# mourisl/Rcorrector

Measured on AMD Instinct MI355X. Metric: corrected reads/sec (150 bp, k=23), higher is better.
Workload: dtype u8/int32/u64

## Files before the change

rcorrector_amd/csrc/rc_correct_core.h:

```cpp
#pragma once
#include "rc_common.h"

#define RC_BS_INLINE 16
#define RC_K(P) (W::KT > 0 ? W::KT : (P).k)

struct rc_run_params {
    int k;
    int max_fix_per_k;
    double error_rate;
    int bad_qual;
    uint32_t bs[RC_BS_INLINE];
    int flags;
    const uint32_t *bs_ext;
    const uint8_t *bound_small;
};
#define RC_BOUND_SMALL 4096
RC_HD uint32_t rc_bs_lookup(const rc_run_params &P, int t)
{
    if (!P.bs[0] || t < 2) return 0;
    if (t < RC_BS_INLINE) return P.bs[t];
    if (!P.bs_ext || t >= RC_BOUND_STEPS) return 0;
    const uint32_t v = P.bs_ext[t];
    return v == RC_BOUND_NEVER ? 0 : v;
}
#define RC_PF_NO_ALT 1

struct rc_island {
    short from, to;
};
struct rc_segment {
    short from, to, lanchor, ranchor;
    int top2[2];
};

struct rc_cnt4 {
    int c0, c1, c2, c3;
};

struct rc_frame {
    uint64_t code;
    int inv;
    int pos;
    int t;
    int threshold;
    int fix_cnt;
    int bottleneck;
    rc_cnt4 cnt;
    int mask;
};

struct rc_read_state {
    unsigned char *base;
    int *counts;
    int *v;
    signed char *path;
    signed char *best;
    unsigned char *strongb;
    unsigned char *polya;
    signed char *qual;
    rc_island *isl;
    rc_segment *seg;
    uint64_t *m_a, *m_t;
    uint64_t *m_n, *m_inv;
    uint64_t *m_x;
    uint32_t *pk;
    int *spec_cnt;
    int *spec_meta;
    int *memo;
    uint64_t *spec_code;
    int *spec_inv;
    int *spec_ret;
    int *spec_keep;
    int *spec_thr;
    int *spec_mask;
    int len, kcnt;
};

#ifndef RC_SPEC
#define RC_SPEC 16
#endif
#define RC_SPEC_ENTRIES 128
#define RC_MEMO_MAX 32

struct rc_spec_state {
    int n;
    int pos;
    int dir;
};

RC_HD int rc_popc64(uint64_t x)
{
#if defined(__HIP_DEVICE_COMPILE__)
    return __popcll(x);
#else
    return __builtin_popcountll(x);
#endif
}
RC_HD int rc_ctz64(uint64_t x)
{
#if defined(__HIP_DEVICE_COMPILE__)
    return __ffsll((long long)x) - 1;
#else
    return __builtin_ctzll(x);
#endif
}
RC_HD int rc_clz64(uint64_t x)
{
#if defined(__HIP_DEVICE_COMPILE__)
    return __clzll((long long)x);
#else
    return __builtin_clzll(x);
#endif
}

RC_HD uint64_t rc_window(const uint64_t *m, int i, int n)
{
    const int w = i >> 6, sh = i & 63;
    uint64_t x = m[w] >> sh;
    if (sh) x |= m[w + 1] << (64 - sh);
    return n >= 64 ? x : (x & ((1ull << n) - 1ull));
}

RC_HD int rc_clz32(uint32_t x)
{
#if defined(__HIP_DEVICE_COMPILE__)
    return __clz((int)x);
#else
    return __builtin_clz(x);
#endif
}

template <class W>
RC_HD void rc_pack_read(W &w, rc_read_state &S)
{
    const int nwords = (S.len + 15) >> 4;
    const uint32_t *b32 = reinterpret_cast<const uint32_t *>(S.base);
    for (int wi = w.lane; wi < nwords; wi += W::STRIDE) {
        uint32_t word = 0;
        for (int q = 0; q < 4; ++q) {
            uint32_t x = b32[4 * wi + q];
            const uint32_t t = (x >> 2) & 0x01010101u;
            x = (x | t | (t << 1)) & 0x03030303u;
            word = (word << 8) | ((x * 0x40100401u) >> 24);
        }
        S.pk[wi] = word;
    }
    w.sync();
}

RC_HD uint64_t rc_code_at(const uint32_t *pk, int p, int n)
{
    const int w0 = p >> 4, sh = 2 * (p & 15);
    uint64_t x = ((uint64_t)pk[w0] << 32) | pk[w0 + 1];
    if (sh) x = (x << sh) | ((uint64_t)pk[w0 + 2] >> (32 - sh));
    return x >> (64 - 2 * n);
}

template <class W>
RC_HD void rc_build_masks(W &w, rc_read_state &S)
{
    const int nw = (S.len + 63) >> 6;
    for (int c = 0; c <= nw; ++c) {
        const int b0 = c << 6;
        const uint64_t ma = w.ballot64(b0, S.len, [&](int i) { return S.base[i] == 0; });
        const uint64_t mt = w.ballot64(b0, S.len, [&](int i) { return S.base[i] == 3; });
        const uint64_t mn = w.ballot64(b0, S.len, [&](int i) { return S.base[i] == 4; });
        const uint64_t mi = w.ballot64(b0, S.len, [&](int i) { return S.base[i] >= 4; });
        S.m_a[c] = ma;
        S.m_t[c] = mt;
        S.m_n[c] = mn;
        S.m_inv[c] = mi;
    }
    w.sync();
}

RC_HD int rc_min(int a, int b) { return a < b ? a : b; }

#define RC_U(x) (w.uni((int)(x)))
#define RC_U64(x) (w.uni64((uint64_t)(x)))

template <class W>
RC_HD int rc_screened(W &w, const rc_read_state &S, int k)
{
    (void)w;
    int n = 0, a = 0, t = 0;
    const int nw = (S.len + 63) >> 6;
    for (int c = 0; c < nw; ++c) {
        n += rc_popc64(S.m_n[c]);
        a += rc_popc64(S.m_a[c]);
        t += rc_popc64(S.m_t[c]);
    }
    return n > 5 || a > S.len - k || t > S.len - k;
}

template <class W>
RC_HD void rc_polya_flags(W &w, rc_read_state &S, int k)
{
    int thr7 = 7;
    if (k / 2 > thr7) thr7 = k / 2;
    for (int i = w.lane; i < S.kcnt; i += W::STRIDE) {
        const int a = rc_popc64(rc_window(S.m_a, i, k));
        const int t = rc_popc64(rc_window(S.m_t, i, k));
        int f = 0;
        if (a >= k - 2 || t >= k - 2) f |= 1;
        if (a >= k - thr7 || t >= k - thr7) f |= 2;
        S.polya[i] = (unsigned char)f;
    }
    w.sync();
}

template <class W>
RC_HD void rc_masked_sorted(W &w, rc_read_state &S)
{
    for (int i = w.lane; i < S.kcnt; i += W::STRIDE) S.v[i] = (S.polya[i] & 2) ? -1 : S.counts[i];
    w.sync();
    w.sort(S.v, S.kcnt);
}

template <class W>
RC_HD int rc_initial_strong(W &w, const rc_read_state &S, int *found, int *prev)
{
    const int kcnt = S.kcnt;
    for (int b0 = ((kcnt - 1) >> 6) << 6; b0 >= 0; b0 -= 64) {
        const uint64_t m = w.ballot64(b0, kcnt, [&](int i) { return i >= 1 && S.v[i] > 2 * S.v[i - 1] && S.v[i] > 10; });
        if (m) {
            const int i = b0 + 63 - rc_clz64(m);
            *found = 1;
            *prev = RC_U(S.v[i - 1]);
            return RC_U(S.v[i]);
        }
    }
    *found = 0;
    *prev = 0;
    int i = kcnt;
    for (int b0 = 0; b0 < kcnt; b0 += 64) {
        const uint64_t m = w.ballot64(b0, kcnt, [&](int j) { return S.v[j] > 0; });
        if (m) {
            i = b0 + rc_ctz64(m);
            break;
        }
    }
    return RC_U(S.v[(i + kcnt - 1) / 2]);
}

template <class W>
RC_HD int rc_front_end(W &w, rc_read_state &S, const rc_run_params &P, int *info)
{
    *info = 4;
    if (S.len < RC_K(P)) return -1;
    if (rc_screened(w, S, RC_K(P))) return -1;
    rc_polya_flags(w, S, RC_K(P));
    rc_masked_sorted(w, S);
    int found, prev;
    int strong = rc_initial_strong(w, S, &found, &prev);
    *info = (found ? 1 : 0) | ((found && prev == 2) ? 2 : 0);
    return strong;
}

struct rc_search_ctx {
    int dir;
    int start, to;
    int max_fix_cnt;
    int best_fix_cnt;
    int best_bottleneck;
    int trial_cnt;
    int top2a, top2b;
};

RC_HD int rc_pin(int x)
{
#if defined(__HIP_DEVICE_COMPILE__)
    return __builtin_amdgcn_readfirstlane(x);
#else
    return x;
#endif
}

RC_HD int rc_sel4(const rc_cnt4 &c, int idx)
{
    const int c0 = rc_pin(c.c0), c1 = rc_pin(c.c1), c2 = rc_pin(c.c2), c3 = rc_pin(c.c3);
    int r = c0;
    r = idx == 1 ? c1 : r;
    r = idx == 2 ? c2 : r;
    r = idx == 3 ? c3 : r;
    return r;
}

RC_HD int rc_candidates(const rc_cnt4 &c, int b, int threshold)
{
    int m = 0;
    if (b != 0 && c.c0 >= threshold) m |= 1;
    if (b != 1 && c.c1 >= threshold) m |= 2;
    if (b != 2 && c.c2 >= threshold) m |= 4;
    if (b != 3 && c.c3 >= threshold) m |= 8;
    return m;
}

RC_HD int rc_pos_threshold(const rc_cnt4 &cnt, int upper, double e)
{
    int mx = 0;
    mx = cnt.c0 > mx ? cnt.c0 : mx;
    mx = cnt.c1 > mx ? cnt.c1 : mx;
    mx = cnt.c2 > mx ? cnt.c2 : mx;
    mx = cnt.c3 > mx ? cnt.c3 : mx;
    int ret = rc_bound_i(mx, e);
    if (ret < 1) ret = 1;
    if (upper > ret || upper <= 0) return ret;
    return upper;
}

RC_HD int rc_max4(const rc_cnt4 &cnt)
{
    int mx = 0;
    mx = cnt.c0 > mx ? cnt.c0 : mx;
    mx = cnt.c1 > mx ? cnt.c1 : mx;
    mx = cnt.c2 > mx ? cnt.c2 : mx;
    mx = cnt.c3 > mx ? cnt.c3 : mx;
    return mx;
}

RC_HD rc_kmer rc_extend(rc_kmer km, int k, int dir, int b)
{
    return dir > 0 ? rc_append(km, k, b) : rc_prepend(km, k, b);
}

RC_HD rc_kmer rc_extend_run(const rc_read_state &S, rc_kmer kc, int k, int dir, int p0, int j)
{
    if (j <= 0) return kc;
    rc_kmer r;
    if (dir > 0) {
        r.code = ((kc.code << (2 * j)) | rc_code_at(S.pk, p0, j)) & rc_kmer_mask(k);
        const uint64_t im = rc_window(S.m_inv, p0, j);
        int inv;
        if (im)
            inv = j - 1 - (63 - rc_clz64(im));
        else
            inv = kc.inv == -1 ? -1 : kc.inv + j;
        r.inv = inv >= k ? -1 : inv;
    } else {
        const int lo = p0 - j + 1;
        if (j >= k)
            r.code = rc_code_at(S.pk, lo, k);
        else
            r.code = (kc.code >> (2 * j)) | (rc_code_at(S.pk, lo, j) << (2 * (k - j)));
        const uint64_t im = rc_window(S.m_inv, lo, j);
        int inv;
        if (im)
            inv = k - 1 - rc_ctz64(im);
        else
            inv = kc.inv == -1 ? -1 : kc.inv - j;
        r.inv = inv < 0 ? -1 : inv;
    }
    return r;
}

template <class W>
RC_HD rc_kmer rc_anchor(W &w, const rc_read_state &S, int k, int a)
{
    rc_kmer kc;
    const int w0 = a >> 4, sh = 2 * (a & 15);
    uint64_t x = ((uint64_t)(uint32_t)RC_U(S.pk[w0]) << 32) | (uint32_t)RC_U(S.pk[w0 + 1]);
    if (sh) x = (x << sh) | ((uint64_t)(uint32_t)RC_U(S.pk[w0 + 2]) >> (32 - sh));
    kc.code = x >> (64 - 2 * k);
    const int mw = a >> 6, ms = a & 63;
    uint64_t im = RC_U64(S.m_inv[mw]) >> ms;
    if (ms) im |= RC_U64(S.m_inv[mw + 1]) << (64 - ms);
    if (k < 64) im &= (1ull << k) - 1ull;
    kc.inv = im ? k - 1 - (63 - rc_clz64(im)) : -1;
    return kc;
}

template <class W>
RC_HD int rc_probe4_cached(W &w, rc_read_state &S, rc_spec_state &Z, const rc_run_params &P, rc_kmer kc, int dir, int pos, int to,
                           rc_cnt4 &cnt)
{
    const int k = RC_K(P);
    if (Z.n > 0 && Z.dir == dir) {
        const int j = (pos - Z.pos) * dir;
        if (j >= 0 && j < Z.n && RC_U64(S.spec_code[j]) == kc.code && RC_U(S.spec_inv[j]) == kc.inv) {
            cnt.c0 = RC_U(S.spec_cnt[4 * j + 0]);
            cnt.c1 = RC_U(S.spec_cnt[4 * j + 1]);
            cnt.c2 = RC_U(S.spec_cnt[4 * j + 2]);
            cnt.c3 = RC_U(S.spec_cnt[4 * j + 3]);
            return j;
        }
    }
    w.stat(3, 1);
    int n = dir > 0 ? (to - pos) : (pos - to + 1);
    if (n > RC_SPEC) n = RC_SPEC;
    if (n < 1) n = 1;
    int am = 0, ana = 0, az = 0, bz = 0;
    const int a0 = dir > 0 ? pos - k : pos + 1;
    if (!(P.flags & RC_PF_NO_ALT) && kc.inv == -1 && a0 >= 0 && a0 + k <= S.len) {
        const rc_kmer o = rc_anchor(w, S, k, a0);
        if (o.code == kc.code && o.inv == -1) {
            const uint64_t zm = w.ballot64(0, n, [&](int j) { return (dir > 0 ? S.counts[pos + j - k + 1] : S.counts[pos - j]) == 0; });
            if (zm) {
                const int z = rc_ctz64(zm), pz = pos + dir * z;
                bz = RC_U(S.base[pz]);
                const int pa = RC_U(dir > 0 ? S.polya[pz - k + 1] : S.polya[pz]);
                const int na = dir > 0 ? to - pz - 1 : pz - to;
                int mm = dir > 0 ? S.len - 1 - pz : pz;
                if (mm > k - 1) mm = k - 1;
                int m = na > mm ? na : mm;
                if (z + 1 + m > 31) m = 31 - (z + 1);
                if (4 * (z + 1) + 3 * m > RC_SPEC_ENTRIES) m = (RC_SPEC_ENTRIES - 4 * (z + 1)) / 3;
                if (bz < 4 && !RC_U(S.strongb[pz]) && !(pa & 1) && na >= 0 && na <= m && m >= 1) {
                    const uint64_t open = w.ballot64(0, na, [&](int j) {
                        const int q = pz + dir * (1 + j);
                        return !S.strongb[q] && !((dir > 0 ? S.polya[q - k + 1] : S.polya[q]) & 1);
                    });
                    if (!open) {
                        am = m;
                        ana = na;
                        az = z;
                        n = z + 1;
                    }
                }
            }
        }
    }
    w.sync();
    const int n4 = 4 * n, E = n4 + 3 * am;
    w.stat(8, E);
    w.stat(9, am > 0 ? 1 : 0);
    auto entry = [&](int e, bool *live) -> rc_kmer {
        rc_kmer km;
        km.code = 0;
        km.inv = 0;
        *live = e < E;
        if (e < n4) {
            const int j = e >> 2, c = e & 3;
            const rc_kmer kj = rc_extend_run(S, kc, k, dir, pos, j);
            if (c == 0) {
                S.spec_code[j] = kj.code;
                S.spec_inv[j] = kj.inv;
            }
            km = rc_extend(kj, k, dir, c);
        } else if (e < E) {
            const int r = e - n4;
            const int a = (r >= am ? 1 : 0) + (r >= 2 * am ? 1 : 0), j = r - a * am;
            const int ca = a + (a >= bz ? 1 : 0);
            km = rc_extend_run(S, kc, k, dir, pos, az + 2 + j);
            if (j + 1 < k) {
                const int sh = dir > 0 ? 2 * (j + 1) : 2 * (k - 1 - (j + 1));
                km.code ^= (uint64_t)(bz ^ ca) << sh;
            }
        }
        return km;
    };
    for (int e0 = 0; e0 < E; e0 += 64) {
        w.for_lanes64(e0, E, [&](int q, int) {
            bool live;
            const rc_kmer km = entry(q, &live);
            S.spec_cnt[q] = w.get(km, dir);
        });
    }
    if (w.lane == 0) {
        S.spec_meta[0] = am;
        S.spec_meta[1] = ana;
        S.spec_meta[2] = az;
    }
    w.sync();
    Z.n = n;
    Z.pos = pos;
    Z.dir = dir;
    cnt.c0 = RC_U(S.spec_cnt[0]);
    cnt.c1 = RC_U(S.spec_cnt[1]);
    cnt.c2 = RC_U(S.spec_cnt[2]);
    cnt.c3 = RC_U(S.spec_cnt[3]);
    return 0;
}

template <class W>
RC_HD int rc_alt_run(W &w, rc_read_state &S, const rc_run_params &P, int a, int dir, rc_kmer &kc, int &pos, int t, int &bottleneck,
                     bool *full)
{
    const int am = RC_U(S.spec_meta[0]), na = RC_U(S.spec_meta[1]), az = RC_U(S.spec_meta[2]);
    *full = na == 0;
    if (na == 0 || t < 1) return 0;
    uint32_t Bt = 0;
    if (dir < 0) {
        Bt = RC_U(rc_bs_lookup(P, t));
        if (!Bt) return 0;
    }
    const int eb = 4 * (az + 1) + a * am;
    const uint64_t okm = w.ballot64(0, na, [&](int j) {
        const int x = S.spec_cnt[eb + j];
        return x >= t && (uint32_t)x >= Bt;
    });
    const uint64_t notok = ~okm;
    int R = notok ? rc_ctz64(notok) : 64;
    if (R > na) R = na;
    if (R == 0) return 0;
    w.for_lanes64(0, R, [&](int j, int) { S.path[pos + dir * j] = -1; });
    bottleneck = rc_min(bottleneck, w.min_range(S.spec_cnt, eb, eb + R));
    rc_kmer nk = rc_extend_run(S, kc, RC_K(P), dir, pos, R);
    kc.code = RC_U64(nk.code);
    kc.inv = RC_U(nk.inv);
    pos += dir * R;
    *full = R == na;
    w.stat(6, 1);
    w.stat(7, R == na ? 1 : 0);
    w.sync();
    return R;
}

template <class W>
RC_HD void rc_search_terminal(W &w, rc_read_state &S, rc_search_ctx &C, const rc_spec_state &Z, int k, int pos, int t, int fix_cnt,
                              int bottleneck, int memo_a)
{
    if (bottleneck < t) ++fix_cnt;
    if (fix_cnt < C.max_fix_cnt) {
        C.top2a = bottleneck;
        C.top2b = -1;
    } else if (fix_cnt == C.max_fix_cnt) {
        if (bottleneck > C.top2a) {
            C.top2b = C.top2a;
            C.top2a = bottleneck;
        } else if (bottleneck > C.top2b) {
            C.top2b = bottleneck;
        }
    }
    if (fix_cnt < C.max_fix_cnt || (fix_cnt == C.max_fix_cnt && bottleneck > C.best_bottleneck)) {
        if (fix_cnt < C.max_fix_cnt) C.trial_cnt = -(C.max_fix_cnt - fix_cnt + 1) * RC_MAX_TRIAL;
        int lo, hi;
        if (C.dir > 0) {
            lo = C.start;
            hi = pos;
        } else {
            lo = pos + 1;
            hi = C.start + 1;
        }
        w.sync();
        for (int i = lo + w.lane; i < hi; i += W::STRIDE) S.best[i] = S.path[i];
        if (memo_a >= 0) {
            const int am = RC_U(S.spec_meta[0]), az = RC_U(S.spec_meta[2]);
            const int pz = Z.pos + C.dir * az, bz = RC_U(S.base[pz]);
            const int ca = memo_a + (memo_a >= bz ? 1 : 0);
            const int eb = 4 * (az + 1) + memo_a * am;
            const int lo_w = C.dir > 0 ? pz - k + 1 : pz - am;
            w.for_lanes64(0, am + 1, [&](int i, int) {
                int c;
                if (C.dir > 0)
                    c = i == 0 ? S.spec_cnt[4 * az + ca] : S.spec_cnt[eb + i - 1];
                else
                    c = i == am ? S.spec_cnt[4 * az + ca] : S.spec_cnt[eb + am - 1 - i];
                S.memo[4 + i] = c;
            });
            if (w.lane == 0) {
                S.memo[0] = am + 1;
                S.memo[1] = lo_w;
                S.memo[2] = pz;
                S.memo[3] = ca;
            }
        }
        w.sync();
        C.max_fix_cnt = fix_cnt;
        C.best_bottleneck = bottleneck;
        C.best_fix_cnt = 1;
    } else if (fix_cnt == C.max_fix_cnt && bottleneck == C.best_bottleneck) {
        C.best_fix_cnt += 1;
    }
}

RC_HD int rc_clamp_threshold(int ret, int upper)
{
    if (upper > ret || upper <= 0) return ret;
    return upper;
}

template <class W>
RC_HD int rc_keep_run(W &w, rc_read_state &S, const rc_run_params &P, const rc_spec_state &Z, int j0, int dir, rc_kmer &kc,
                      int &pos, int &t, int fix_cnt, int &bottleneck, int &sp)
{
    const int k = RC_K(P);
    const int n = Z.n;
    w.for_lanes64(j0, n, [&](int jj, int) {
        const int c0 = S.spec_cnt[4 * jj], c1 = S.spec_cnt[4 * jj + 1], c2 = S.spec_cnt[4 * jj + 2], c3 = S.spec_cnt[4 * jj + 3];
        int mx = 0;
        mx = c0 > mx ? c0 : mx;
        mx = c1 > mx ? c1 : mx;
        mx = c2 > mx ? c2 : mx;
        mx = c3 > mx ? c3 : mx;
        int ret = rc_bound_i(mx, P.error_rate);
        if (ret < 1) ret = 1;
        S.spec_ret[jj] = rc_clamp_threshold(ret, t);
        const int b = S.base[Z.pos + dir * jj];
        int kc2 = -1;
        kc2 = b == 0 ? c0 : kc2;
        kc2 = b == 1 ? c1 : kc2;
        kc2 = b == 2 ? c2 : kc2;
        kc2 = b == 3 ? c3 : kc2;
        S.spec_keep[jj] = kc2;
    });
    w.sync();
    if (dir > 0) {
        w.for_lanes64(j0, n, [&](int jj, int) { S.spec_thr[jj] = S.spec_ret[jj]; });
    } else {
        w.prefix_min(S.spec_ret, S.spec_thr, j0, n);
    }
    w.sync();
    const uint64_t okm = w.ballot64(j0, n, [&](int jj) { return S.spec_keep[jj] >= S.spec_thr[jj]; });
    const uint64_t notok = ~okm;
    int R = notok ? rc_ctz64(notok) : 64;
    if (R > n - j0) R = n - j0;
    w.stat(0, 1);
    w.stat(1, R);
    w.stat(2, n - j0);
    if (R == 0) return 0;
    const uint64_t fm = w.ballot64(j0, j0 + R, [&](int jj) {
        const int p2 = Z.pos + dir * jj;
        const int b = S.base[p2];
        const int pa = dir > 0 ? S.polya[p2 - k + 1] : S.polya[p2];
        int m2 = 0;
        if (!S.strongb[p2] && !(pa & 1)) {
            const int thr = S.spec_thr[jj];
            for (int c = 0; c < 4; ++c)
                if (c != b && S.spec_cnt[4 * jj + c] >= thr) m2 |= 1 << c;
        }
        S.spec_mask[jj] = m2;
        S.path[p2] = -1;
        return m2 != 0;
    });
    w.sync();
    uint64_t f2 = fm;
    while (f2) {
        const int jj = j0 + rc_ctz64(f2);
        f2 &= f2 - 1;
        rc_frame f;
        f.code = RC_U64(S.spec_code[jj]);
        f.inv = RC_U(S.spec_inv[jj]);
        f.pos = Z.pos + dir * jj;
        f.t = (dir > 0 || jj == j0) ? t : RC_U(S.spec_thr[jj - 1]);
        f.threshold = RC_U(S.spec_thr[jj]);
        f.fix_cnt = fix_cnt;
        int bb = bottleneck;
        for (int i = j0; i < jj; ++i) bb = rc_min(bb, RC_U(S.spec_keep[i]));
        f.bottleneck = bb;
        f.cnt.c0 = RC_U(S.spec_cnt[4 * jj + 0]);
        f.cnt.c1 = RC_U(S.spec_cnt[4 * jj + 1]);
        f.cnt.c2 = RC_U(S.spec_cnt[4 * jj + 2]);
        f.cnt.c3 = RC_U(S.spec_cnt[4 * jj + 3]);
        f.mask = RC_U(S.spec_mask[jj]);
        w.stack_push(sp, f);
        ++sp;
    }
    const int idx = j0 + R;
    bottleneck = rc_min(bottleneck, w.min_range(S.spec_keep, j0, idx));
    if (dir < 0) t = RC_U(S.spec_thr[idx - 1]);
    if (idx < n) {
        kc.code = RC_U64(S.spec_code[idx]);
        kc.inv = RC_U(S.spec_inv[idx]);
    } else {
        rc_kmer last;
        last.code = RC_U64(S.spec_code[idx - 1]);
        last.inv = RC_U(S.spec_inv[idx - 1]);
        kc = rc_extend(last, k, dir, RC_U(S.base[Z.pos + dir * (idx - 1)]));
    }
    pos = Z.pos + dir * idx;
    return R;
}

template <class W>
RC_HD void rc_search(W &w, rc_read_state &S, const rc_run_params &P, rc_search_ctx &C, rc_kmer kc0,
                     int t0)
{
    const int k = RC_K(P);
    const int dir = C.dir;
    int sp = 0;
    rc_kmer kc = kc0;
    int pos = C.start, t = t0, fix_cnt = 0, bottleneck = 1000000000;
    bool have = true;
    rc_spec_state Z;
    Z.n = 0;
    Z.pos = 0;
    Z.dir = dir;
    int alt_a = -1;
    auto alt_of = [&](uint64_t code, int inv, int p, int c) -> int {
        if (Z.n <= 0 || RC_U(S.spec_meta[0]) <= 0) return -1;
        const int az = RC_U(S.spec_meta[2]);
        if (p != Z.pos + dir * az || RC_U64(S.spec_code[az]) != code || RC_U(S.spec_inv[az]) != inv) return -1;
        const int bz = RC_U(S.base[p]);
        return c < bz ? c : c - 1;
    };

    for (;;) {
        w.phase(8);
        if (!have) {
            if (sp == 0) break;
            rc_frame f;
            w.stack_top(sp - 1, f);
            int c = 0;
            while (!((f.mask >> c) & 1)) ++c;
            f.mask &= ~(1 << c);
            if (f.mask == 0)
                --sp;
            else
                w.stack_set_mask(sp - 1, f.mask);
            rc_kmer fk;
            fk.code = f.code;
            fk.inv = f.inv;
            S.path[f.pos] = (signed char)c;
            w.sync();
            ++C.trial_cnt;
            alt_a = alt_of(f.code, f.inv, f.pos, c);
            kc = rc_extend(fk, k, dir, c);
            pos = f.pos + dir;
            t = dir > 0 ? f.t : f.threshold;
            fix_cnt = f.fix_cnt + (RC_U(S.base[f.pos]) < 4 ? 1 : 0);
            bottleneck = rc_min(f.bottleneck, rc_sel4(f.cnt, c));
            have = true;
        }

        if (C.trial_cnt > RC_MAX_TRIAL) {
            if (C.max_fix_cnt > 2) {
                --C.max_fix_cnt;
                C.best_fix_cnt = 0;
                C.best_bottleneck = -1;
                C.trial_cnt = 0;
            } else {
                have = false;
                continue;
            }
        }
        if (fix_cnt > C.max_fix_cnt) {
            have = false;
            alt_a = -1;
            continue;
        }
        int memo_a = -1;
        if (alt_a >= 0) {
            bool full;
            rc_alt_run(w, S, P, alt_a, dir, kc, pos, t, bottleneck, &full);
            if (full) memo_a = alt_a;
            alt_a = -1;
        }
        if (dir > 0 ? (pos >= C.to) : (pos < C.to)) {
            w.phase(14);
            rc_search_terminal(w, S, C, Z, k, pos, t, fix_cnt, bottleneck, memo_a);
            have = false;
            continue;
        }

        rc_cnt4 cnt;
        w.phase(9);
        const int j0 = rc_probe4_cached(w, S, Z, P, kc, dir, pos, C.to, cnt);
        w.phase(10);
        if (rc_keep_run(w, S, P, Z, j0, dir, kc, pos, t, fix_cnt, bottleneck, sp) > 0) {
            have = true;
            continue;
        }
        w.phase(11);
        int threshold = RC_U(rc_pos_threshold(cnt, t, P.error_rate));
        const int b = RC_U(S.base[pos]);
        const bool bvalid = b < 4;

        int mask = 0;
        {
            const int pa = RC_U(dir > 0 ? S.polya[pos - k + 1] : S.polya[pos]);
            if (!RC_U(S.strongb[pos]) && !(pa & 1)) mask = rc_candidates(cnt, b, threshold);
        }

        bool first = false;
        rc_kmer nkc = kc;
        int npos = pos, nt = t, nfix = fix_cnt, nbott = bottleneck;
        if (bvalid) {
            int c0 = rc_sel4(cnt, b);
            if (c0 >= threshold) {
                S.path[pos] = -1;
                nkc = rc_extend(kc, k, dir, b);
                npos = pos + dir;
                nt = dir > 0 ? t : threshold;
                nbott = rc_min(bottleneck, c0);
                first = true;
            } else if (threshold == 1 && t <= 2) {
                w.phase(12);
                rc_kmer tmp = rc_extend(kc, k, dir, b);
                int m = dir > 0 ? (C.to - 1 - pos) : (pos - C.to);
                if (m > k - 1) m = k - 1;
                int steps = k, i = pos;
                (void)c0;
                if (m > 0) {
                    const rc_kmer tmp0 = tmp;
                    int mc = Z.n - 1 - j0;
                    if (mc > m) mc = m;
                    int sN = 0;
                    if (mc > 0) {
                        const uint64_t hit = w.ballot64(1, mc + 1, [&](int q) { return S.spec_keep[j0 + q] >= threshold; });
                        if (hit) sN = 1 + rc_ctz64(hit);
                    }
                    if (sN == 0 && m > mc) {
                        const uint64_t hit = w.ballot64(mc + 1, m + 1, [&](int q) {
                            return w.get(rc_extend_run(S, tmp0, k, dir, pos + dir, q), dir) >= threshold;
                        });
                        w.stat(4, 1);
                        w.stat(5, m - mc);
                        if (hit) sN = mc + 1 + rc_ctz64(hit);
                    }
                    if (sN > 0) {
                        tmp = rc_extend_run(S, tmp0, k, dir, pos + dir, sN);
                        tmp.code = RC_U64(tmp.code);
                        tmp.inv = RC_U(tmp.inv);
                        i = pos + dir * sN;
                        steps = sN;
                    }
                }
                if (steps < k && (dir > 0 ? (i < C.to) : (i >= C.to))) {
                    int lo = dir > 0 ? pos : i, hi = dir > 0 ? i : pos;
                    for (int j = lo + w.lane; j <= hi; j += W::STRIDE) S.path[j] = -1;
                    nkc = tmp;
                    npos = i + dir;
                    nt = dir > 0 ? t : threshold;
                    nfix = fix_cnt + 1;
                    first = true;
                }
            }
        }

        if (!first && mask) {
            int c = 0;
            while (!((mask >> c) & 1)) ++c;
            mask &= ~(1 << c);
            S.path[pos] = (signed char)c;
            ++C.trial_cnt;
            alt_a = alt_of(kc.code, kc.inv, pos, c);
            nkc = rc_extend(kc, k, dir, c);
            npos = pos + dir;
            nt = dir > 0 ? t : threshold;
            nfix = fix_cnt + (bvalid ? 1 : 0);
            nbott = rc_min(bottleneck, rc_sel4(cnt, c));
            first = true;
        }

        if (first) {
            if (mask) {
                rc_frame f;
                f.code = kc.code;
                f.inv = kc.inv;
                f.pos = pos;
                f.t = t;
                f.threshold = threshold;
                f.fix_cnt = fix_cnt;
                f.bottleneck = bottleneck;
                f.cnt = cnt;
                f.mask = mask;
                w.stack_push(sp, f);
                ++sp;
            }
        } else {
            w.phase(13);
            rc_kmer tmp = kc;
            int i, c1 = 0;
            int thr = threshold;
            if (dir > 0) {
                for (i = pos; i < C.to; ++i) {
                    rc_cnt4 cn;
                    if (i == pos)
                        cn = cnt;
                    else
                        rc_probe4_cached(w, S, Z, P, tmp, dir, i, C.to, cn);
                    thr = RC_U(rc_pos_threshold(cn, t, P.error_rate));
                    int bb = RC_U(S.base[i]);
                    tmp = rc_append(tmp, k, bb);
                    c1 = (bb < 4) ? rc_sel4(cn, bb) : 0;
                    S.path[i] = -1;
                    if (c1 >= thr) break;
                }
                int pen = (i < S.len) ? (i - pos - k + 1) : ((i - pos) / 2);
                if (pen <= 0) pen = 1;
                nfix = fix_cnt + pen;
                if (i >= C.to) i -= 1;
                npos = i + 1;
                nt = t;
            } else {
                for (i = pos; i >= C.to; --i) {
                    rc_cnt4 cn;
                    if (i == pos)
                        cn = cnt;
                    else
                        rc_probe4_cached(w, S, Z, P, tmp, dir, i, C.to, cn);
                    thr = RC_U(rc_pos_threshold(cn, t, P.error_rate));
                    int bb = RC_U(S.base[i]);
                    tmp = rc_prepend(tmp, k, bb);
                    c1 = (bb < 4) ? rc_sel4(cn, bb) : 0;
                    S.path[i] = -1;
                    if (c1 >= thr) break;
                }
                int pen = (i >= 0) ? (pos - i - k + 1) : (pos - 1);
                if (pen <= 0) pen = 1;
                nfix = fix_cnt + pen;
                if (i <= C.to) ++i;
                npos = i - 1;
                nt = thr;
            }
            nkc = tmp;
            nbott = bottleneck;
        }
        w.sync();
        kc = nkc;
        pos = npos;
        t = nt;
        fix_cnt = nfix;
        bottleneck = nbott;
        have = true;
    }
}

template <class W>
RC_HD int rc_correct_read(W &w, rc_read_state &S, const rc_run_params &P, int pair_t, int strong0,
                          int info0)
{
    const int k = RC_K(P);
    const int len = S.len, kcnt = S.kcnt;
    if (w.lane == 0) S.memo[0] = 0;
    if (len < k) return -1;
    if (info0 & 4) return -1;
    w.trace_passed();

    int strong = strong0, trust;
    bool flag = false;
    trust = RC_U(rc_bound_i(strong, P.error_rate));
    if (info0 & 1) {
        if (strong >= 20 && (info0 & 2) && trust < 3) {
            flag = true;
            trust = 3;
        }
    }
    if (pair_t >= 1 && strong > pair_t) {
        if (!flag || pair_t < 20) trust = RC_U(rc_bound_i(pair_t, P.error_rate));
        strong = pair_t;
    }
    if (trust < 2) trust = 2;

    int iter = 0, total_fix = 0, bad_segment_cnt = 0;
    int tstart = 0, tend = 0;
    for (;;) {
        w.phase(2);
        w.trace_iter(strong, trust);
        const int allowed_fix = len;
        total_fix = 0;
        bool unfixable = false, force_next = false;
        int isl_cnt = 0, longest = -1, j = 0, i;

        for (i = w.lane; i < len; i += W::STRIDE) {
            S.strongb[i] = 0;
            S.path[i] = -1;
        }
        w.sync();

        {
            const int nwk = (kcnt + 63) >> 6;
            for (int c = 0; c <= nwk; ++c) {
                const uint64_t tm = w.ballot64(c << 6, kcnt, [&](int q) { return S.counts[q] >= strong && !(S.polya[q] & 1); });
                S.m_x[c] = tm;
            }
            w.sync();
            int *rs = S.v;
            int *re = S.v + (kcnt + 1) / 2 + 1;
            int ns = 0, ne = 0;
            for (int c = 0; c < nwk; ++c) {
                const uint64_t T = RC_U64(S.m_x[c]);
                const uint64_t prev = c ? (RC_U64(S.m_x[c - 1]) >> 63) : 0ull;
                const uint64_t next = RC_U64(S.m_x[c + 1]) & 1ull;
                uint64_t st = T & ~((T << 1) | prev);
                uint64_t en = T & ~((T >> 1) | (next << 63));
                while (st) {
                    rs[ns++] = (c << 6) + rc_ctz64(st);
                    st &= st - 1;
                }
                while (en) {
                    re[ne++] = (c << 6) + rc_ctz64(en);
                    en &= en - 1;
                }
            }
            w.sync();
            if (!(RC_U64(S.m_x[0]) & 1ull)) {
                longest = 0;
                tstart = 0;
                tend = -1;
            }
            for (int r = 0; r < ns; ++r) {
                const int f = RC_U(rs[r]), t2 = RC_U(re[r]);
                j = t2 - f + 1;
                if (j > longest) {
                    longest = j;
                    tstart = f;
                    tend = t2;
                }
                if (j >= 2) {
                    S.isl[isl_cnt].from = (short)f;
                    S.isl[isl_cnt].to = (short)t2;
                    ++isl_cnt;
                }
            }
            w.sync();
        }

        for (i = 1; i < isl_cnt; ++i) {
            int pf = RC_U(S.isl[i - 1].from), pt = RC_U(S.isl[i - 1].to), cf = RC_U(S.isl[i].from), ct = RC_U(S.isl[i].to);
            if (cf <= pt + k) {
                int len1 = pt - pf, len2 = ct - cf, overlap = pt + k - cf;
                const uint64_t weak = w.ballot64(pt + 1, cf, [&](int q) { return S.counts[q] <= 2 && S.counts[q] < trust; });
                if (!weak) continue;
                if (overlap > 3) continue;
                if (len1 < len2)
                    S.isl[i - 1].to = (short)(pt - (overlap + 1));
                else
                    S.isl[i].from = (short)(cf + (overlap + 1));
                w.sync();
            }
        }

        {
            int nb = 0, cura = 0, curb = -2;
            for (i = 0; i < isl_cnt; ++i) {
                const int f = RC_U(S.isl[i].from), tt = RC_U(S.isl[i].to);
                if (f > tt) continue;
                const int a2 = f, b2 = tt + k - 1;
                for (j = a2 + w.lane; j <= b2; j += W::STRIDE) S.strongb[j] = 1;
                if (nb > 0 && a2 <= curb + 1) {
                    if (b2 > curb) curb = b2;
                } else {
                    if (nb > 0) {
                        S.isl[nb - 1].from = (short)cura;
                        S.isl[nb - 1].to = (short)curb;
                    }
                    cura = a2;
                    curb = b2;
                    ++nb;
                }
            }
            if (nb > 0) {
                S.isl[nb - 1].from = (short)cura;
                S.isl[nb - 1].to = (short)curb;
            }
            isl_cnt = nb;
        }
        if (isl_cnt == 0) {
            S.isl[0].from = (short)tstart;
            S.isl[0].to = (short)(tend + k - 1);
            isl_cnt = 1;
        }
        w.sync();

        int seg_cnt = 0;
        {
            int f0 = RC_U(S.isl[0].from), t0 = RC_U(S.isl[0].to);
            if (f0 > 0) {
                S.seg[seg_cnt].from = 0;
                S.seg[seg_cnt].to = (short)(f0 - 1);
                S.seg[seg_cnt].lanchor = 0;
                S.seg[seg_cnt].ranchor = (short)(t0 - f0 + 1);
                ++seg_cnt;
            }
            for (i = 0; i < isl_cnt - 1; ++i) {
                int af = RC_U(S.isl[i].from), at = RC_U(S.isl[i].to), bf = RC_U(S.isl[i + 1].from), bt = RC_U(S.isl[i + 1].to);
                S.seg[seg_cnt].from = (short)(at + 1);
                S.seg[seg_cnt].to = (short)(bf - 1);
                S.seg[seg_cnt].lanchor = (short)(at - af + 1);
                S.seg[seg_cnt].ranchor = (short)(bt - bf + 1);
                ++seg_cnt;
            }
            int lf = RC_U(S.isl[i].from), lt = RC_U(S.isl[i].to);
            if (lt < len - 1) {
                S.seg[seg_cnt].from = (short)(lt + 1);
                S.seg[seg_cnt].to = (short)len;
                S.seg[seg_cnt].lanchor = (short)(lt - lf + 1);
                S.seg[seg_cnt].ranchor = 0;
                ++seg_cnt;
            }
            for (i = 0; i < seg_cnt; ++i) S.seg[i].top2[0] = S.seg[i].top2[1] = -1;
        }
        w.sync();
        w.trace_strong(S.strongb, len);

        if (longest == -1) return -1;
        if (longest == kcnt) return 0;
#if defined(RC_EXP_STOP) && RC_EXP_STOP == 3
        return 0;
#endif

        for (i = w.lane; i < len; i += W::STRIDE) S.best[i] = -1;
        w.sync();
        bad_segment_cnt = 0;
        w.phase(3);
        if (seg_cnt > 0) {
            rc_search_ctx C;
            int best_bottleneck = RC_INF;
            C.best_fix_cnt = -1;
            C.trial_cnt = 0;
            C.max_fix_cnt = allowed_fix;
            for (int si = 0; si < seg_cnt; ++si) {
                const int sf = RC_U(S.seg[si].from), st = RC_U(S.seg[si].to);
                C.top2a = C.top2b = -1;
                C.trial_cnt = 0;
                C.max_fix_cnt = (st - sf + 1) * P.max_fix_per_k / k * 2 + 1;
                if (C.max_fix_cnt < P.max_fix_per_k) C.max_fix_cnt = P.max_fix_per_k;
                C.best_bottleneck = -1;
                int a;
                if (RC_U(S.seg[si].lanchor) >= RC_U(S.seg[si].ranchor)) {
                    int extend = (st == len) ? 0 : (k - 1);
                    a = sf - k;
                    if (a < 0) return -1;
                    C.dir = 1;
                    C.start = a + k;
                    C.to = st + extend;
                } else {
                    int extend = (sf == 0) ? 0 : (k - 1);
                    a = st + 1;
                    if (a + k > len) return -1;
                    C.dir = -1;
                    C.start = a - 1;
                    C.to = sf - extend;
                }
                rc_search(w, S, P, C, rc_anchor(w, S, k, a), trust);
                w.phase(3);
                S.seg[si].top2[0] = C.top2a;
                S.seg[si].top2[1] = C.top2b;
                w.sync();
                if (C.best_bottleneck == -1) {
                    ++bad_segment_cnt;
                    continue;
                }
                if (C.best_bottleneck < best_bottleneck) best_bottleneck = C.best_bottleneck;
                if (best_bottleneck == -1) break;
                if (C.trial_cnt > RC_MAX_TRIAL) return -1;
                total_fix += C.max_fix_cnt;
            }
            int best_fix_cnt = C.best_fix_cnt;
            if (best_bottleneck != -1) {
                best_fix_cnt = 1;
                for (i = 0; i < seg_cnt; ++i)
                    if (RC_U(S.seg[i].top2[1]) >= best_bottleneck) best_fix_cnt *= 2;
            }
            if (best_bottleneck != -1 && iter == 0 &&
                RC_U(rc_less_than_bound(best_bottleneck, strong, P.error_rate) ? 1 : 0))
                force_next = true;
            if (best_fix_cnt >= 2)
                return -1;
            else if (best_fix_cnt <= 0)
                unfixable = true;
        }
        if (total_fix == 0 && force_next) return 0;
        if (total_fix > allowed_fix) unfixable = true;
        if (!unfixable && !force_next) break;
        if (trust < 10 && !force_next) return -1;

        w.phase(4);
        rc_masked_sorted(w, S);
        bool has_drop = false;
        i = 0;
        for (int b0 = ((kcnt - 1) >> 6) << 6; b0 >= 0; b0 -= 64) {
            const int st = strong;
            const uint64_t dm = w.ballot64(b0, kcnt, [&](int q) {
                if (q < 1) return false;
                const int vi = S.v[q], vp = S.v[q - 1];
                return vi <= st && ((vi > 2 * vp && vi > 10) || (vp == 0 && vi >= 5));
            });
            const uint64_t bm = dm & w.ballot64(b0, kcnt, [&](int q) { return S.v[q] < st; });
            if (bm) {
                has_drop = true;
                i = b0 + 63 - rc_clz64(bm);
                break;
            }
            if (dm) has_drop = true;
        }
        if (has_drop) {
            ++iter;
            int vi = RC_U(S.v[i]);
            trust = RC_U(rc_bound_i(vi, P.error_rate));
            strong = vi;
        } else
            break;
    }

    w.phase(5);
#if defined(RC_EXP_STOP) && RC_EXP_STOP == 4
    return total_fix;
#endif
    int cnt = 0;
    for (int b0 = 0; b0 < len; b0 += 64) {
        const uint64_t fm = w.ballot64(b0, len, [&](int q) { return S.base[q] != 4 && S.best[q] != -1; });
        if (fm) {
            w.for_lanes64(b0, len, [&](int q, int ln) {
                if ((fm >> ln) & 1ull) S.v[cnt + rc_popc64(fm & ((1ull << ln) - 1ull))] = q;
            });
            cnt += rc_popc64(fm);
        }
    }
    w.sync();
    const int badq = P.bad_qual;
    const int q0 = RC_U(S.qual[0]);
    for (int i = 1; i < cnt; ++i) {
        const int pi = RC_U(S.v[i]), pp = RC_U(S.v[i - 1]);
        if (q0 != 0 && (RC_U(S.qual[pi]) <= badq && RC_U(S.qual[pp]) <= badq)) continue;
        if (pi - pp + 1 > k) continue;
        int lo = pp - k + 1;
        if (lo < 0) lo = 0;
        if (i >= 2) {
            const int pprev = RC_U(S.v[i - 2]);
            if (lo < pprev + 1) lo = pprev + 1;
        }
        int hi = kcnt;
        if (i < cnt - 1) {
            const int pnext = RC_U(S.v[i + 1]);
            if (hi > pnext - k + 1) hi = pnext - k + 1;
        }
        uint32_t ms = 0xFFFFFFFFu, md = 0xFFFFFFFFu;
        w.for_lanes64(pp - k + 1, hi, [&](int j, int) {
            if (j < lo || j > pi) return;
            const uint32_t c = (uint32_t)S.counts[j];
            if (j + k - 1 >= pi && j <= pp)
                md = c < md ? c : md;
            else
                ms = c < ms ? c : ms;
        });
        ms = w.wave_min_u32(ms);
        md = w.wave_min_u32(md);
        if (ms == 0xFFFFFFFFu || md == 0xFFFFFFFFu) continue;
        const int min_single = (int)ms, min_double = (int)md;
        if (min_single > 1 && min_double > 1 && min_single > min_double / 2 && min_single < 2 * min_double) {
            S.best[pi] = -1;
            S.best[pp] = -1;
            for (int jj = i - 2; jj >= 0 && RC_U(S.v[jj + 1]) - RC_U(S.v[jj]) + 1 <= k; --jj) S.best[RC_U(S.v[jj])] = -1;
            while (i + 1 < cnt && RC_U(S.v[i + 1]) - RC_U(S.v[i]) + 1 <= k) {
                S.best[RC_U(S.v[i + 1])] = -1;
                ++i;
            }
            w.sync();
        }
    }

    if (total_fix > 3 && len > 10) {
        int tmp = rc_popc64(w.ballot64(0, 10, [&](int q) { return S.best[q] != -1 && S.base[q] != 4 && (int)S.qual[q] > badq; }));
        if (tmp >= 2)
            w.for_lanes64(0, 10, [&](int q, int) {
                if (S.base[q] != 4) S.best[q] = -1;
            });
        w.sync();
        tmp = rc_popc64(w.ballot64(len - 10, len, [&](int q) { return S.best[q] != -1 && S.base[q] != 4 && (int)S.qual[q] > badq; }));
        if (tmp >= 3)
            w.for_lanes64(len - 10, len, [&](int q, int) {
                if (S.base[q] != 4) S.best[q] = -1;
            });
        w.sync();
    }

    if (total_fix >= P.max_fix_per_k) {
        const int nw = (len + 63) >> 6;
        for (int c = 0; c <= nw; ++c) {
            const uint64_t f = w.ballot64(c << 6, len, [&](int q) { return S.base[q] != 4 && S.best[q] != -1; });
            const uint64_t g = f & w.ballot64(c << 6, len, [&](int q) { return (int)S.qual[q] > badq; });
            S.m_a[c] = f;
            S.m_t[c] = g;
        }
        w.sync();
        int bad = 0;
        for (int i = w.lane; i < kcnt; i += W::STRIDE)
            if (rc_popc64(rc_window(S.m_a, i, k)) + rc_popc64(rc_window(S.m_t, i, k)) > 2 * P.max_fix_per_k) bad = 1;
        if (w.reduce_add(bad)) return -1;
    }

    int ret = 0;
    for (int i = w.lane; i < len; i += W::STRIDE)
        if (S.best[i] != -1) ++ret;
    ret = w.reduce_add(ret);
    if (ret == 0 && bad_segment_cnt > 0) return -1;
    return ret;
}

template <class W>
RC_HD int rc_select_kth(W &w, const int *v, int n, int kth, uint32_t hi)
{
    uint32_t prefix = 0;
    for (int b = 31 - rc_clz32(hi | 1u); b >= 0; --b) {
        const uint32_t cand = prefix | (1u << b);
        int below = 0;
        for (int b0 = 0; b0 < n; b0 += 64) below += rc_popc64(w.ballot64(b0, n, [&](int q) { return (uint32_t)v[q] < cand; }));
        if (below <= kth) prefix = cand;
    }
    return (int)prefix;
}

template <class W>
RC_HD void rc_kmer_info(W &w, rc_read_state &S, const rc_run_params &P, int ret, int *l, int *m,
                        int *h)
{
    const int k = RC_K(P);
    *l = *m = *h = 0;
    if (S.kcnt <= 0) return;
    const int nw = (S.len + 63) >> 6;
    for (int c = 0; c <= nw; ++c) {
        uint64_t fm = 0;
        if (ret > 0) fm = w.ballot64(c << 6, S.len, [&](int q) { return S.best[q] != -1; });
        S.m_x[c] = fm;
    }
    w.sync();
    int memo_n = 0, memo_lo = 0, memo_p = 0;
    if (ret > 0) {
        memo_n = RC_U(S.memo[0]);
        if (memo_n > 0) {
            memo_lo = RC_U(S.memo[1]);
            memo_p = RC_U(S.memo[2]);
            if (RC_U(S.best[memo_p]) != RC_U(S.memo[3])) memo_n = 0;
        }
    }
    int nvalid = 0;
    uint32_t lo = 0xFFFFFFFFu, hi = 0;
    for (int b0 = 0; b0 < S.kcnt; b0 += 64) {
        const uint64_t vm = w.ballot64(b0, S.kcnt, [&](int q) {
            return (rc_window(S.m_inv, q, k) & ~rc_window(S.m_x, q, k)) == 0;
        });
        nvalid += rc_popc64(vm);
        w.for_lanes64(b0, S.kcnt, [&](int q, int ln) {
            uint32_t c = 0xFFFFFFFFu;
            if ((vm >> ln) & 1ull) {
                int cc;
                const uint64_t fw = ret > 0 ? rc_window(S.m_x, q, k) : 0ull;
                if (fw != 0) {
                    const int d = memo_p - q;
                    if (q >= memo_lo && q < memo_lo + memo_n && d >= 0 && d < k && fw == (1ull << d))
                        cc = S.memo[4 + q - memo_lo];
                    else
                        cc = w.lookup(rc_code_at(S.pk, q, k));
                } else
                    cc = S.counts[q];
                if (cc == 0) cc = 1;
                c = (uint32_t)cc;
                lo = c < lo ? c : lo;
                hi = c > hi ? c : hi;
            }
            S.v[q] = (int)c;
        });
    }
    w.sync();
    if (nvalid == 0) return;
    lo = w.wave_min_u32(lo);
    hi = w.wave_max_u32(hi);
    *l = (int)lo;
    *h = (int)hi;
    *m = rc_select_kth(w, S.v, S.kcnt, nvalid / 2, hi);
}
```

rcorrector_amd/csrc/rc_correct_kernel.h:

```cpp
#pragma once
#include <cstddef>
#include <cstdio>
#include <cstdlib>

#include "rc_internal.h"
#include "rc_device.h"

template <bool PROF, bool TRACE = false, bool SORT_REGS = true, int KT_ = 0>
struct DevWaveT {
    static const int STRIDE = 64;
    static constexpr int KT = KT_;
    int lane;
    unsigned long long t_last = 0;
    int cur_phase = 0;
    unsigned long long *acc = nullptr;
#ifdef RC_EXP_ROUNDS
    int rounds = 0;
    __device__ __forceinline__ void stat(int i, int v)
    {
        if (i == 3) rounds += v;
    }
#else
    int rounds = 0, rounds_max = 0;
    long long rounds_sum = 0;
    long long stv[10] = {0, 0, 0, 0, 0, 0, 0, 0, 0, 0};
    __device__ __forceinline__ void stat(int i, int v)
    {
        if (PROF && i == 3) rounds += v;
        if (PROF && i != 3 && i < 10) stv[i] += v;
    }
#endif
    int32_t *tr = nullptr;
    int tr_cap = 0;
    __device__ __forceinline__ void trace_passed()
    {
        if (TRACE && lane == 0) tr[0] |= 1;
    }
    __device__ __forceinline__ void trace_iter(int strong, int trust)
    {
        if (TRACE) {
            const int it = uni(tr[1]);
            if (lane == 0) {
                if (it < tr_cap) {
                    int32_t *e = tr + 2 + (size_t)it * RC_TRACE_WORDS;
                    e[0] = strong;
                    e[1] = trust;
                    e[2] = 0;
                    e[3] = 0;
                }
                tr[1] = it + 1;
            }
            sync();
        }
    }
    __device__ __forceinline__ void trace_strong(const unsigned char *strongb, int len)
    {
        if (TRACE) {
            const int it = uni(tr[1]) - 1;
            if (it >= 0 && it < tr_cap) {
                int32_t *e = tr + 2 + (size_t)it * RC_TRACE_WORDS;
                for (int c = 0; c < RC_MAX_READ_LENGTH / 64; ++c) {
                    const uint64_t m = ballot64(c << 6, len, [&](int q) { return strongb[q] != 0; });
                    if (lane == 0) {
                        e[4 + 2 * c] = (int32_t)(uint32_t)m;
                        e[5 + 2 * c] = (int32_t)(uint32_t)(m >> 32);
                    }
                }
                if (lane == 0) e[2] = 1;
            }
            sync();
        }
    }
    __device__ __forceinline__ int uni(int x) { return __builtin_amdgcn_readfirstlane(x); }
    __device__ __forceinline__ uint64_t uni64(uint64_t x)
    {
        const uint32_t lo = (uint32_t)__builtin_amdgcn_readfirstlane((int)(uint32_t)x);
        const uint32_t hi = (uint32_t)__builtin_amdgcn_readfirstlane((int)(uint32_t)(x >> 32));
        return ((uint64_t)hi << 32) | lo;
    }
    __device__ __forceinline__ void phase(int id)
    {
        if (id < 8) asm volatile("" : "+v"(lane));
        if (PROF) {
            unsigned long long t = __builtin_readcyclecounter();
            if (lane == 0) acc[cur_phase] += t - t_last;
            t_last = t;
            cur_phase = id;
        }
    }
    rc_table_view T;
    int k;
    rc_frame *stack;

    __device__ __forceinline__ void sync()
    {
        __builtin_amdgcn_fence(__ATOMIC_RELEASE, "wavefront");
        __builtin_amdgcn_wave_barrier();
        __builtin_amdgcn_fence(__ATOMIC_ACQUIRE, "wavefront");
    }

    template <class F>
    __device__ __forceinline__ uint64_t ballot64(int base, int n, F pred)
    {
        const int i = base + lane;
        bool p = false;
        if (i < n) p = pred(i);
        return __ballot(p);
    }
    template <class F>
    __device__ __forceinline__ void for_lanes64(int base, int n, F body)
    {
        const int i = base + lane;
        if (i < n) body(i, lane);
    }

    __device__ __forceinline__ int reduce_add(int x)
    {
#pragma unroll
        for (int o = 32; o > 0; o >>= 1) x += __shfl_xor(x, o, 64);
        return __builtin_amdgcn_readfirstlane(x);
    }

    template <bool MAX>
    __device__ __forceinline__ uint32_t wave_minmax_u32(uint32_t x)
    {
        auto op = [](uint32_t a, uint32_t b) { return MAX ? (a > b ? a : b) : (a < b ? a : b); };
        x = op(x, (uint32_t)__builtin_amdgcn_update_dpp(0, (int)x, 0xB1, 0xF, 0xF, true));
        x = op(x, (uint32_t)__builtin_amdgcn_update_dpp(0, (int)x, 0x4E, 0xF, 0xF, true));
        x = op(x, (uint32_t)__builtin_amdgcn_update_dpp(0, (int)x, 0x141, 0xF, 0xF, true));
        x = op(x, (uint32_t)__builtin_amdgcn_update_dpp(0, (int)x, 0x140, 0xF, 0xF, true));
        const uint32_t r0 = (uint32_t)__builtin_amdgcn_readlane((int)x, 0), r1 = (uint32_t)__builtin_amdgcn_readlane((int)x, 16);
        const uint32_t r2 = (uint32_t)__builtin_amdgcn_readlane((int)x, 32), r3 = (uint32_t)__builtin_amdgcn_readlane((int)x, 48);
        return op(op(r0, r1), op(r2, r3));
    }
    __device__ __forceinline__ uint32_t wave_min_u32(uint32_t x) { return wave_minmax_u32<false>(x); }
    __device__ __forceinline__ uint32_t wave_max_u32(uint32_t x) { return wave_minmax_u32<true>(x); }

    __device__ __forceinline__ void prefix_min(const int *in, int *out, int j0, int n)
    {
        const bool live = lane >= j0 && lane < n;
        int x = live ? in[lane] : 2147483647;
        auto step = [&](int y) { x = y < x ? y : x; };
        step(__builtin_amdgcn_update_dpp(2147483647, x, 0x111, 0xF, 0xF, false));
        step(__builtin_amdgcn_update_dpp(2147483647, x, 0x112, 0xF, 0xF, false));
        step(__builtin_amdgcn_update_dpp(2147483647, x, 0x114, 0xF, 0xF, false));
        step(__builtin_amdgcn_update_dpp(2147483647, x, 0x118, 0xF, 0xF, false));
        if (n > 16) {
            const int r0 = __builtin_amdgcn_readlane(x, 15), r1 = __builtin_amdgcn_readlane(x, 31), r2 = __builtin_amdgcn_readlane(x, 47);
            const int m01 = r0 < r1 ? r0 : r1, m012 = m01 < r2 ? m01 : r2;
            const int row = lane >> 4;
            const int before = row == 0 ? 2147483647 : (row == 1 ? r0 : (row == 2 ? m01 : m012));
            x = before < x ? before : x;
        }
        if (live) out[lane] = x;
    }
    __device__ __forceinline__ int min_range(const int *a, int lo, int hi)
    {
        const int i = lo + lane;
        const uint32_t x = i < hi ? ((uint32_t)a[i] ^ 0x80000000u) : 0xFFFFFFFFu;
        return (int)(wave_min_u32(x) ^ 0x80000000u);
    }

    uint32_t n_req = 0;
    uint32_t n_probe = 0, n_absent = 0;
    __device__ __forceinline__ int get(rc_kmer km, int dir = 0)
    {
        if (km.inv != -1) return 0;
        const uint64_t rv = rc_revcomp(km.code, KT ? KT : k);
        const uint64_t canon = rv < km.code ? rv : km.code;
        const int c = rc_table_lookup_o<true, true>(T, canon, dir > 0 ? km.code : (dir < 0 ? rv : canon), PROF ? &n_req : nullptr);
        if (PROF) {
            ++n_probe;
            n_absent += c == 0 ? 1u : 0u;
        }
        return c;
    }

    __device__ __forceinline__ int lookup(uint64_t code) { return rc_table_lookup(T, rc_canonical(code, KT ? KT : k), PROF ? &n_req : nullptr); }

    template <int E>
    __device__ __forceinline__ void bitonic_regs(int *a, int n)
    {
        int x[E];
#pragma unroll
        for (int e = 0; e < E; ++e) {
            const int g = e * 64 + lane;
            x[e] = g < n ? a[g] : 2147483647;
        }
#pragma unroll
        for (int size = 2; size <= E * 64; size <<= 1) {
#pragma unroll
            for (int stride = size >> 1; stride > 0; stride >>= 1) {
                if (stride >= 64) {
#pragma unroll
                    for (int e = 0; e < E; ++e) {
                        const int pe = e ^ (stride >> 6);
                        if (pe > e) {
                            const bool up = ((e * 64) & size) == 0;
                            const int lo = x[e] < x[pe] ? x[e] : x[pe];
                            const int hi = x[e] < x[pe] ? x[pe] : x[e];
                            x[e] = up ? lo : hi;
                            x[pe] = up ? hi : lo;
                        }
                    }
                } else {
#pragma unroll
                    for (int e = 0; e < E; ++e) {
                        const int g = e * 64 + lane;
                        const int y = __shfl_xor(x[e], stride, 64);
                        const bool up = (g & size) == 0;
                        const bool lower = (lane & stride) == 0;
                        const int lo = x[e] < y ? x[e] : y;
                        const int hi = x[e] < y ? y : x[e];
                        x[e] = (up == lower) ? lo : hi;
                    }
                }
            }
        }
        sync();
#pragma unroll
        for (int e = 0; e < E; ++e) {
            const int g = e * 64 + lane;
            if (g < n) a[g] = x[e];
        }
        sync();
    }

    __device__ __forceinline__ void sort(int *a, int n)
    {
        if (SORT_REGS) {
            if (n <= 64) return bitonic_regs<1>(a, n);
            if (n <= 128) return bitonic_regs<2>(a, n);
            if (n <= 256) return bitonic_regs<4>(a, n);
        }
        int n2 = 1;
        while (n2 < n) n2 <<= 1;
        for (int i = n + lane; i < n2; i += 64) a[i] = 2147483647;
        sync();
        for (int size = 2; size <= n2; size <<= 1) {
            for (int stride = size >> 1; stride > 0; stride >>= 1) {
                for (int t = lane; t < (n2 >> 1); t += 64) {
                    const int pos = 2 * t - (t & (stride - 1));
                    const int par = pos + stride;
                    const bool up = (pos & size) == 0;
                    const int x = a[pos], y = a[par];
                    if ((x > y) == up) {
                        a[pos] = y;
                        a[par] = x;
                    }
                }
                sync();
            }
        }
    }

    uint32_t *lstack = nullptr;
    int lstack_n = 0;
    static constexpr int FRAME_DWORDS = (int)(sizeof(rc_frame) / 4);
    __device__ __forceinline__ void stack_push(int sp, const rc_frame &f)
    {
        if (sp < lstack_n) {
            if (lane == 0) {
                uint32_t *d = lstack + sp * FRAME_DWORDS;
                d[0] = (uint32_t)f.code;
                d[1] = (uint32_t)(f.code >> 32);
                d[2] = (uint32_t)f.inv;
                d[3] = (uint32_t)f.pos;
                d[4] = (uint32_t)f.t;
                d[5] = (uint32_t)f.threshold;
                d[6] = (uint32_t)f.fix_cnt;
                d[7] = (uint32_t)f.bottleneck;
                d[8] = (uint32_t)f.cnt.c0;
                d[9] = (uint32_t)f.cnt.c1;
                d[10] = (uint32_t)f.cnt.c2;
                d[11] = (uint32_t)f.cnt.c3;
                d[12] = (uint32_t)f.mask;
            }
            sync();
            return;
        }
        if (lane == 0) stack[sp] = f;
        __threadfence_block();
    }
    __device__ __forceinline__ void stack_top(int idx, rc_frame &f)
    {
        static_assert(sizeof(rc_frame) == 56 && offsetof(rc_frame, mask) == 48, "rc_frame layout");
        uint32_t d[13];
        if (idx < lstack_n) {
            const uint32_t *p = lstack + idx * FRAME_DWORDS;
#pragma unroll
            for (int q = 0; q < 13; ++q) d[q] = p[q];
        } else {
            const uint32_t *p = reinterpret_cast<const uint32_t *>(stack + idx);
#pragma unroll
            for (int q = 0; q < 13; ++q) d[q] = __hip_atomic_load(p + q, __ATOMIC_RELAXED, __HIP_MEMORY_SCOPE_WORKGROUP);
        }
        f.code = ((uint64_t)(uint32_t)uni((int)d[1]) << 32) | (uint32_t)uni((int)d[0]);
        f.inv = uni((int)d[2]);
        f.pos = uni((int)d[3]);
        f.t = uni((int)d[4]);
        f.threshold = uni((int)d[5]);
        f.fix_cnt = uni((int)d[6]);
        f.bottleneck = uni((int)d[7]);
        f.cnt.c0 = uni((int)d[8]);
        f.cnt.c1 = uni((int)d[9]);
        f.cnt.c2 = uni((int)d[10]);
        f.cnt.c3 = uni((int)d[11]);
        f.mask = uni((int)d[12]);
    }
    __device__ __forceinline__ void stack_set_mask(int idx, int mask)
    {
        if (idx < lstack_n) {
            if (lane == 0) lstack[idx * FRAME_DWORDS + 12] = (uint32_t)mask;
            sync();
            return;
        }
        if (lane == 0) stack[idx].mask = mask;
        __threadfence_block();
    }
};
typedef DevWaveT<false> DevWave;

#ifndef RC_DEQUEUE
#define RC_DEQUEUE 8
#endif
#define RC_META_WORDS 6

struct rc_lds_layout {
    int cap, cap2;
    size_t o_counts, o_v, o_isl, o_seg, o_base, o_path, o_best, o_strongb, o_polya, o_qual, o_masks, o_spec, o_pk, o_meta, total;
    int mask_words;
};

static __host__ __device__ constexpr inline int rc_seg_capacity(int cap) { return cap <= 192 ? 20 : cap / 6 + 4; }

static __host__ __device__ constexpr inline rc_lds_layout rc_layout(int cap)
{
    rc_lds_layout L{};
    L.cap = cap;
    int c2 = 64;
    while (c2 < cap) c2 <<= 1;
    L.cap2 = c2;
    const int nseg = rc_seg_capacity(cap);
    const int nisl = cap / 3 + 2;
    size_t o = 0;
    L.mask_words = cap / 64 + 2;
    L.o_masks = o;
    o += (size_t)L.mask_words * 8 * 5;
    L.o_spec = o;
    o += (size_t)RC_SPEC_ENTRIES * 4 + (size_t)RC_SPEC * (8 + 4 + 4 * 4) + 16 + (size_t)(4 + RC_MEMO_MAX) * 4;
    L.o_pk = o;
    o += (size_t)(cap / 16 + 4) * 4;
    L.o_meta = o;
    o += (size_t)RC_DEQUEUE * RC_META_WORDS * 4;
    L.o_counts = o;
    o += (size_t)cap * 4;
    L.o_v = o;
    o += (size_t)c2 * 4;
    L.o_seg = o;
    o += (size_t)nseg * sizeof(rc_segment);
    if ((size_t)nisl * sizeof(rc_island) <= (size_t)RC_SPEC_ENTRIES * 4 + (size_t)RC_SPEC * 8) {
        L.o_isl = L.o_spec;
    } else {
        L.o_isl = o;
        o += (size_t)nisl * sizeof(rc_island);
    }
    o = (o + 15) & ~(size_t)15;
    L.o_base = o;
    o += cap;
    L.o_path = o;
    o += cap;
    L.o_best = o;
    o += cap;
    L.o_strongb = o;
    o += cap;
    L.o_polya = o;
    o += cap;
    L.o_qual = o;
    o += cap;
    L.total = (o + 15) & ~(size_t)15;
    return L;
}

__device__ __forceinline__ void rc_carve(uint8_t *lds, const rc_lds_layout &L, rc_read_state &S)
{
    S.counts = reinterpret_cast<int *>(lds + L.o_counts);
    S.v = reinterpret_cast<int *>(lds + L.o_v);
    S.seg = reinterpret_cast<rc_segment *>(lds + L.o_seg);
    S.isl = reinterpret_cast<rc_island *>(lds + L.o_isl);
    S.base = lds + L.o_base;
    S.path = reinterpret_cast<signed char *>(lds + L.o_path);
    S.best = reinterpret_cast<signed char *>(lds + L.o_best);
    S.strongb = lds + L.o_strongb;
    S.polya = lds + L.o_polya;
    S.qual = reinterpret_cast<signed char *>(lds + L.o_qual);
    uint64_t *mm = reinterpret_cast<uint64_t *>(lds + L.o_masks);
    S.m_a = mm;
    S.m_t = mm + L.mask_words;
    S.m_n = mm + 2 * L.mask_words;
    S.m_inv = mm + 3 * L.mask_words;
    S.m_x = mm + 4 * L.mask_words;
    S.pk = reinterpret_cast<uint32_t *>(lds + L.o_pk);
    S.spec_code = reinterpret_cast<uint64_t *>(lds + L.o_spec);
    S.spec_cnt = reinterpret_cast<int *>(lds + L.o_spec + RC_SPEC * 8);
    S.spec_inv = S.spec_cnt + RC_SPEC_ENTRIES;
    S.spec_ret = S.spec_inv + RC_SPEC;
    S.spec_keep = S.spec_ret + RC_SPEC;
    S.spec_thr = S.spec_keep + RC_SPEC;
    S.spec_mask = S.spec_thr + RC_SPEC;
    S.spec_meta = S.spec_mask + RC_SPEC;
    S.memo = S.spec_meta + 4;
}

struct rc_kernel_args {
    rc_table_view T;
    rc_run_params P;
    int mode;
    uint32_t n;
    uint8_t *seq;
    size_t nbytes;
    const uint8_t *qual;
    int qual_bits;
    uint32_t qual_split, qual_base2;
    const uint32_t *off;
    const int32_t *counts;
    int32_t *strong, *info;
    uint8_t *cls;
    uint8_t *cand;
    uint2 *runs;
    const uint32_t *worklist;
    const uint32_t *n_work;
    int32_t *ret, *l, *m, *h;
    rc_frame *stack;
    int stack_frames;
    uint32_t *work;
    int cap;
    int cap_class;
    unsigned long long *phase_cycles;
    int32_t *rounds_out;
    uint32_t work_stride;
    int fused_front_end;
    int32_t *trace;
    int trace_cap;
    int tier_lo, tier_hi;
    int pair_override;
};
__device__ __forceinline__ int rc_unit_max_len(const rc_kernel_args &A, uint32_t r, int len)
{
    if (A.mode == 0) return len;
    const uint32_t half = A.n >> 1, mr = A.mode == 1 ? (r < half ? r + half : r - half) : (r ^ 1u);
    const int ml = (int)(A.off[mr + 1] - A.off[mr]) - 1;
    return ml > len ? ml : len;
}
__device__ __forceinline__ bool rc_in_tier(const rc_kernel_args &A, int unit_max_len) { return unit_max_len > A.tier_lo && unit_max_len <= A.tier_hi; }

template <class W>
__device__ __forceinline__ void rc_load_read(W &w, const rc_kernel_args &A, rc_read_state &S, uint32_t o, int len, int lane, bool with_qual)
{
    S.len = len;
    S.kcnt = len >= RC_K(A.P) ? len - RC_K(A.P) + 1 : 0;
    for (int i = lane; i < len; i += 64) {
        S.base[i] = (unsigned char)rc_base_code(A.seq[o + i]);
        S.counts[i] = i < S.kcnt ? A.counts[o + i] : 0;
        if (with_qual) S.qual[i] = rc_qual_at(A.qual, A.qual_bits, A.qual_split, A.qual_base2, o + (uint32_t)i);
    }
    w.sync();
    rc_build_masks(w, S);
    rc_pack_read(w, S);
}

#ifndef RC_HEADS
#define RC_HEADS 8
#endif
#ifndef RC_K3_WAVES
#define RC_K3_WAVES 8
#endif

static __host__ __device__ constexpr int rc_k3_waves(int cap)
{
    const int by_lds = cap <= 192 ? 8 : (cap <= 320 ? 5 : 1);
    return by_lds < RC_K3_WAVES ? by_lds : RC_K3_WAVES;
}

template <int CAP, bool PROF, bool TRACE, int KT = 0, int TL = 0>
__global__ __launch_bounds__(64, rc_k3_waves(CAP)) void k_correct(rc_kernel_args A)
{
    constexpr rc_lds_layout L = rc_layout(CAP);
    __shared__ __attribute__((aligned(16))) uint8_t lds[L.total + (PROF ? 128 : 0)];
    rc_read_state S;
    rc_carve(lds, L, S);
    typedef DevWaveT<PROF, TRACE, false, KT> W;
    W w;
    w.lane = threadIdx.x;
    w.tr_cap = A.trace_cap;
    if (PROF) {
        w.acc = reinterpret_cast<unsigned long long *>(lds + L.total);
        if (w.lane < 16) w.acc[w.lane] = 0;
        w.sync();
        w.t_last = __builtin_readcyclecounter();
    }
    w.T = A.T;
    if (TL != 0) w.T.layout = 1;
    if (TL == 1) w.T.ext = 0;
    if (KT != 0) w.T.k = KT;
    w.k = A.P.k;
    w.stack = A.stack + (size_t)blockIdx.x * A.stack_frames;
    w.lstack = reinterpret_cast<uint32_t *>(S.v);
    w.lstack_n = (int)((size_t)L.cap2 * 4 / sizeof(rc_frame));
    if (PROF && w.lane == 0) atomicMin(A.phase_cycles + 8, (unsigned long long)wall_clock64());
    const int n_sections = A.n_work ? RC_WORK_CLASSES : 1;
    int section = 0;
    uint32_t n_work = A.n_work ? (uint32_t)__builtin_amdgcn_readfirstlane((int)A.n_work[0]) : A.n;
    const uint32_t *list = A.worklist;
    uint32_t *heads = A.work;
    uint32_t chunk_lo = 0, chunk_hi = 0, chunk_base = 0;
    uint32_t *meta = reinterpret_cast<uint32_t *>(lds + L.o_meta);
    int head = (int)(blockIdx.x % RC_HEADS), heads_done = 0;
    for (;;) {
        if (chunk_lo >= chunk_hi) {
            bool got = false;
            for (;;) {
                while (heads_done < RC_HEADS) {
                    const uint32_t lo = (uint32_t)(((uint64_t)n_work * (uint32_t)head) / RC_HEADS);
                    const uint32_t hi = (uint32_t)(((uint64_t)n_work * (uint32_t)(head + 1)) / RC_HEADS);
                    uint32_t r0 = hi - lo;
                    if (hi > lo) {
                        if (w.lane == 0) r0 = atomicAdd(heads + head * 32, (uint32_t)RC_DEQUEUE);
                        r0 = (uint32_t)__builtin_amdgcn_readfirstlane((int)r0);
                    }
                    if (r0 < hi - lo) {
                        chunk_lo = lo + r0;
                        chunk_hi = hi - chunk_lo > (uint32_t)RC_DEQUEUE ? chunk_lo + RC_DEQUEUE : hi;
                        got = true;
                        break;
                    }
                    head = head + 1 == RC_HEADS ? 0 : head + 1;
                    ++heads_done;
                }
                if (got || ++section >= n_sections) break;
                n_work = (uint32_t)__builtin_amdgcn_readfirstlane((int)A.n_work[section]);
                list = A.worklist + (size_t)section * A.work_stride;
                heads = A.work + section * (RC_HEADS * 32);
                head = (int)(blockIdx.x % RC_HEADS);
                heads_done = 0;
            }
            if (!got) {
                if (PROF && w.lane == 0) atomicMin(A.phase_cycles + 9, (unsigned long long)wall_clock64());
                break;
            }
            chunk_base = chunk_lo;
            if ((uint32_t)w.lane < chunk_hi - chunk_lo) {
                uint32_t ri = chunk_lo + (uint32_t)w.lane;
                if (list) ri = list[ri];
                uint32_t *mw = meta + w.lane * RC_META_WORDS;
                mw[0] = ri;
                mw[1] = A.off[ri];
                mw[2] = A.off[ri + 1];
                if (!A.fused_front_end) {
                    mw[3] = (uint32_t)A.strong[ri];
                    mw[4] = (uint32_t)A.info[ri];
                    if (A.mode == 1) {
                        const uint32_t half = A.n >> 1;
                        mw[5] = (uint32_t)A.strong[ri < half ? ri + half : ri - half];
                    } else if (A.mode == 2)
                        mw[5] = (uint32_t)A.strong[ri ^ 1u];
                }
            }
            w.sync();
        }
        const int ci = (int)(chunk_lo - chunk_base);
        ++chunk_lo;
        const uint32_t *me = meta + ci * RC_META_WORDS;
        const uint32_t r = (uint32_t)w.uni((int)me[0]);
        const uint32_t o = (uint32_t)w.uni((int)me[1]);
        w.phase(0);
        if (TRACE) {
            w.tr = A.trace + (size_t)r * (2 + (size_t)A.trace_cap * RC_TRACE_WORDS);
            if (w.lane == 0) w.tr[0] = w.tr[1] = 0;
            w.sync();
        }
#if defined(RC_EXP_STOP) && RC_EXP_STOP == 0
        if (w.lane == 0) A.ret[r] = (int)o;
        continue;
#endif
        rc_load_read(w, A, S, o, w.uni((int)(me[2] - o) - 1), w.lane, true);
#if defined(RC_EXP_STOP) && RC_EXP_STOP == 1
        if (w.lane == 0) A.ret[r] = (int)S.m_inv[0] + (int)S.pk[1] + S.counts[5] + S.qual[7];
        w.sync();
        continue;
#endif
        int strong0, info0;
        if (A.fused_front_end) {
            w.phase(1);
            strong0 = rc_front_end(w, S, A.P, &info0);
        } else {
            strong0 = w.uni((int)me[3]);
            info0 = w.uni((int)me[4]);
        }
        int pair_t = A.pair_override;
        if (A.mode != 0) pair_t = rc_min(strong0, w.uni((int)me[5]));
        w.phase(1);
        if (!A.fused_front_end && S.kcnt > 0 && !(info0 & 4)) rc_polya_flags(w, S, RC_K(A.P));
#if defined(RC_EXP_STOP) && RC_EXP_STOP == 2
        if (w.lane == 0) A.ret[r] = (int)S.polya[3] + pair_t;
        w.sync();
        continue;
#endif
        const int ret = rc_correct_read(w, S, A.P, pair_t, strong0, info0);
#if defined(RC_EXP_STOP) && (RC_EXP_STOP == 3 || RC_EXP_STOP == 4 || RC_EXP_STOP == 5)
        if (w.lane == 0) A.ret[r] = ret + S.best[3] + S.seg[0].from;
        w.sync();
        continue;
#endif
        w.phase(6);
        w.sync();
        if (ret > 0) {
            for (int i = w.lane; i < S.len; i += 64) {
                const int f = S.best[i];
                if (f != -1) {
                    A.seq[o + i] = (uint8_t)("ACGT"[f]);
                    S.base[i] = (unsigned char)f;
                }
            }
            w.sync();
            rc_pack_read(w, S);
        }
        int l, m, h;
        rc_kmer_info(w, S, A.P, ret, &l, &m, &h);
        if (w.lane == 0) {
            A.ret[r] = ret;
#ifdef RC_EXP_ROUNDS
            A.l[r] = w.rounds;
            w.rounds = 0;
#else
            A.l[r] = l;
#endif
            A.m[r] = m;
            A.h[r] = h;
        }
        w.sync();
        w.phase(7);
#ifndef RC_EXP_ROUNDS
        if (PROF) {
            if (A.rounds_out && w.lane == 0) A.rounds_out[r] = w.rounds;
            w.rounds_sum += w.rounds;
            w.rounds_max = w.rounds > w.rounds_max ? w.rounds : w.rounds_max;
            w.rounds = 0;
        }
#endif
    }
    if (PROF && w.lane == 0) {
        w.phase(7);
        for (int i = 0; i < 8; ++i) atomicAdd(A.phase_cycles + i, w.acc[i]);
        for (int i = 8; i < 16; ++i) atomicAdd(A.phase_cycles + 8 + i, w.acc[i]);
        atomicMax(A.phase_cycles + 10, (unsigned long long)wall_clock64());
#ifndef RC_EXP_ROUNDS
        atomicAdd(A.phase_cycles + 11, (unsigned long long)w.rounds_sum);
        atomicMax(A.phase_cycles + 12, (unsigned long long)w.rounds_max);
        for (int i = 0; i < 10; ++i)
            if (i != 3) atomicAdd(A.phase_cycles + 24 + i, (unsigned long long)w.stv[i]);
#endif
    }
    if (PROF) {
        const int req = w.reduce_add((int)w.n_req), prb = w.reduce_add((int)w.n_probe), abs_ = w.reduce_add((int)w.n_absent);
        if (w.lane == 0) {
            atomicAdd(A.phase_cycles + 13, (unsigned long long)(uint32_t)req);
            atomicAdd(A.phase_cycles + 14, (unsigned long long)(uint32_t)prb);
            atomicAdd(A.phase_cycles + 15, (unsigned long long)(uint32_t)abs_);
        }
    }
}

typedef void (*rc_k3_launcher)(dim3 grid, hipStream_t stream, const rc_kernel_args &A);
rc_k3_launcher rc_k3_special(int k, int layout, int ext);
#define RC_K3_SPECIAL(KT, TL)                                                                                     \
    void rc_k3_launch_##KT##_##TL(dim3 grid, hipStream_t stream, const rc_kernel_args &A)                          \
    {                                                                                                             \
        hipLaunchKernelGGL((k_correct<192, false, false, KT, TL>), grid, dim3(64), 0, stream, A);                  \
    }
```

Measured before the change: 367.2 million.

## Spill dequeue state to LDS descriptor and reload params via wave accessor to cut registers

Moves the per-wave work-queue state (chunk bounds, section/head cursor, current meta index) out of live registers into a small LDS descriptor block. It also routes run-parameter accesses through a wave-provided params accessor, so kernel arguments are re-read from their constant source instead of being held across the long correction routine. The aim is to lower VGPR/SGPR pressure in the large correction kernel and so raise occupancy or avoid spills. The cost is extra LDS reads and writes plus readfirstlane broadcasts on each read iteration.

```diff
diff --git a/rcorrector_amd/csrc/rc_correct_core.h b/rcorrector_amd/csrc/rc_correct_core.h
--- a/rcorrector_amd/csrc/rc_correct_core.h
+++ b/rcorrector_amd/csrc/rc_correct_core.h
@@ -82,6 +82,82 @@
 #define RC_SPEC_ENTRIES 128
 #define RC_MEMO_MAX 32
 
+enum {
+    RC_D_CHUNK_LO = 0,
+    RC_D_CHUNK_HI,
+    RC_D_CHUNK_BASE,
+    RC_D_QUEUE,
+    RC_D_META,
+    RC_D_WORDS = 8
+};
+RC_HD constexpr int rc_desc_queue(int section, int head, int heads_done) { return section | (head << 8) | (heads_done << 16); }
+RC_HD constexpr int rc_desc_section(int q) { return q & 0xFF; }
+RC_HD constexpr int rc_desc_head(int q) { return (q >> 8) & 0xFF; }
+RC_HD constexpr int rc_desc_heads_done(int q) { return (q >> 16) & 0xFF; }
+
+#ifndef RC_DEQUEUE
+#define RC_DEQUEUE 8
+#endif
+#define RC_META_WORDS 6
+
+struct rc_lds_layout {
+    int cap, cap2;
+    size_t o_counts, o_v, o_isl, o_seg, o_base, o_path, o_best, o_strongb, o_polya, o_qual, o_masks, o_spec, o_pk, o_meta, o_desc, total;
+    int mask_words;
+};
+
+RC_HD constexpr int rc_seg_capacity(int cap) { return cap <= 192 ? 20 : cap / 6 + 4; }
+
+RC_HD constexpr rc_lds_layout rc_layout(int cap)
+{
+    rc_lds_layout L{};
+    L.cap = cap;
+    int c2 = 64;
+    while (c2 < cap) c2 <<= 1;
+    L.cap2 = c2;
+    const int nseg = rc_seg_capacity(cap);
+    const int nisl = cap / 3 + 2;
+    size_t o = 0;
+    L.mask_words = cap / 64 + 2;
+    L.o_masks = o;
+    o += (size_t)L.mask_words * 8 * 5;
+    L.o_spec = o;
+    o += (size_t)RC_SPEC_ENTRIES * 4 + (size_t)RC_SPEC * (8 + 4 + 4 * 4) + 16 + (size_t)(4 + RC_MEMO_MAX) * 4;
+    L.o_pk = o;
+    o += (size_t)(cap / 16 + 4) * 4;
+    L.o_meta = o;
+    o += (size_t)RC_DEQUEUE * RC_META_WORDS * 4;
+    L.o_desc = o;
+    o += (size_t)RC_D_WORDS * 4;
+    L.o_counts = o;
+    o += (size_t)cap * 4;
+    L.o_v = o;
+    o += (size_t)c2 * 4;
+    L.o_seg = o;
+    o += (size_t)nseg * sizeof(rc_segment);
+    if ((size_t)nisl * sizeof(rc_island) <= (size_t)RC_SPEC_ENTRIES * 4 + (size_t)RC_SPEC * 8) {
+        L.o_isl = L.o_spec;
+    } else {
+        L.o_isl = o;
+        o += (size_t)nisl * sizeof(rc_island);
+    }
+    o = (o + 15) & ~(size_t)15;
+    L.o_base = o;
+    o += cap;
+    L.o_path = o;
+    o += cap;
+    L.o_best = o;
+    o += cap;
+    L.o_strongb = o;
+    o += cap;
+    L.o_polya = o;
+    o += cap;
+    L.o_qual = o;
+    o += cap;
+    L.total = (o + 15) & ~(size_t)15;
+    return L;
+}
+
 struct rc_spec_state {
     int n;
     int pos;
@@ -178,6 +254,18 @@
 
 #define RC_U(x) (w.uni((int)(x)))
 #define RC_U64(x) (w.uni64((uint64_t)(x)))
+
+template <class W>
+RC_HD auto rc_params_(W &w, const rc_run_params &P, int) -> decltype(w.params(P))
+{
+    return w.params(P);
+}
+template <class W>
+RC_HD const rc_run_params &rc_params_(W &, const rc_run_params &P, long)
+{
+    return P;
+}
+#define RC_P (rc_params_(w, P, 0))
 
 template <class W>
 RC_HD int rc_screened(W &w, const rc_read_state &S, int k)
@@ -391,7 +479,7 @@
     if (n < 1) n = 1;
     int am = 0, ana = 0, az = 0, bz = 0;
     const int a0 = dir > 0 ? pos - k : pos + 1;
-    if (!(P.flags & RC_PF_NO_ALT) && kc.inv == -1 && a0 >= 0 && a0 + k <= S.len) {
+    if (!(RC_P.flags & RC_PF_NO_ALT) && kc.inv == -1 && a0 >= 0 && a0 + k <= S.len) {
         const rc_kmer o = rc_anchor(w, S, k, a0);
         if (o.code == kc.code && o.inv == -1) {
             const uint64_t zm = w.ballot64(0, n, [&](int j) { return (dir > 0 ? S.counts[pos + j - k + 1] : S.counts[pos - j]) == 0; });
@@ -481,7 +569,7 @@
     if (na == 0 || t < 1) return 0;
     uint32_t Bt = 0;
     if (dir < 0) {
-        Bt = RC_U(rc_bs_lookup(P, t));
+        Bt = RC_U(rc_bs_lookup(RC_P, t));
         if (!Bt) return 0;
     }
     const int eb = 4 * (az + 1) + a * am;
@@ -583,7 +671,7 @@
         mx = c1 > mx ? c1 : mx;
         mx = c2 > mx ? c2 : mx;
         mx = c3 > mx ? c3 : mx;
-        int ret = rc_bound_i(mx, P.error_rate);
+        int ret = rc_bound_i(mx, RC_P.error_rate);
         if (ret < 1) ret = 1;
         S.spec_ret[jj] = rc_clamp_threshold(ret, t);
         const int b = S.base[Z.pos + dir * jj];
@@ -752,7 +840,7 @@
             continue;
         }
         w.phase(11);
-        int threshold = RC_U(rc_pos_threshold(cnt, t, P.error_rate));
+        int threshold = RC_U(rc_pos_threshold(cnt, t, RC_P.error_rate));
         const int b = RC_U(S.base[pos]);
         const bool bvalid = b < 4;
 
@@ -860,7 +948,7 @@
                         cn = cnt;
                     else
                         rc_probe4_cached(w, S, Z, P, tmp, dir, i, C.to, cn);
-                    thr = RC_U(rc_pos_threshold(cn, t, P.error_rate));
+                    thr = RC_U(rc_pos_threshold(cn, t, RC_P.error_rate));
                     int bb = RC_U(S.base[i]);
                     tmp = rc_append(tmp, k, bb);
                     c1 = (bb < 4) ? rc_sel4(cn, bb) : 0;
@@ -880,7 +968,7 @@
                         cn = cnt;
                     else
                         rc_probe4_cached(w, S, Z, P, tmp, dir, i, C.to, cn);
-                    thr = RC_U(rc_pos_threshold(cn, t, P.error_rate));
+                    thr = RC_U(rc_pos_threshold(cn, t, RC_P.error_rate));
                     int bb = RC_U(S.base[i]);
                     tmp = rc_prepend(tmp, k, bb);
                     c1 = (bb < 4) ? rc_sel4(cn, bb) : 0;
@@ -920,7 +1008,7 @@
 
     int strong = strong0, trust;
     bool flag = false;
-    trust = RC_U(rc_bound_i(strong, P.error_rate));
+    trust = RC_U(rc_bound_i(strong, RC_P.error_rate));
     if (info0 & 1) {
         if (strong >= 20 && (info0 & 2) && trust < 3) {
             flag = true;
@@ -928,7 +1016,7 @@
         }
     }
     if (pair_t >= 1 && strong > pair_t) {
-        if (!flag || pair_t < 20) trust = RC_U(rc_bound_i(pair_t, P.error_rate));
+        if (!flag || pair_t < 20) trust = RC_U(rc_bound_i(pair_t, RC_P.error_rate));
         strong = pair_t;
     }
     if (trust < 2) trust = 2;
@@ -1095,8 +1183,8 @@
                 const int sf = RC_U(S.seg[si].from), st = RC_U(S.seg[si].to);
                 C.top2a = C.top2b = -1;
                 C.trial_cnt = 0;
-                C.max_fix_cnt = (st - sf + 1) * P.max_fix_per_k / k * 2 + 1;
-                if (C.max_fix_cnt < P.max_fix_per_k) C.max_fix_cnt = P.max_fix_per_k;
+                C.max_fix_cnt = (st - sf + 1) * RC_P.max_fix_per_k / k * 2 + 1;
+                if (C.max_fix_cnt < RC_P.max_fix_per_k) C.max_fix_cnt = RC_P.max_fix_per_k;
                 C.best_bottleneck = -1;
                 int a;
                 if (RC_U(S.seg[si].lanchor) >= RC_U(S.seg[si].ranchor)) {
@@ -1135,7 +1223,7 @@
                     if (RC_U(S.seg[i].top2[1]) >= best_bottleneck) best_fix_cnt *= 2;
             }
             if (best_bottleneck != -1 && iter == 0 &&
-                RC_U(rc_less_than_bound(best_bottleneck, strong, P.error_rate) ? 1 : 0))
+                RC_U(rc_less_than_bound(best_bottleneck, strong, RC_P.error_rate) ? 1 : 0))
                 force_next = true;
             if (best_fix_cnt >= 2)
                 return -1;
@@ -1169,7 +1257,7 @@
         if (has_drop) {
             ++iter;
             int vi = RC_U(S.v[i]);
-            trust = RC_U(rc_bound_i(vi, P.error_rate));
+            trust = RC_U(rc_bound_i(vi, RC_P.error_rate));
             strong = vi;
         } else
             break;
@@ -1190,7 +1278,7 @@
         }
     }
     w.sync();
-    const int badq = P.bad_qual;
+    const int badq = RC_P.bad_qual;
     const int q0 = RC_U(S.qual[0]);
     for (int i = 1; i < cnt; ++i) {
         const int pi = RC_U(S.v[i]), pp = RC_U(S.v[i - 1]);
@@ -1247,7 +1335,7 @@
         w.sync();
     }
 
-    if (total_fix >= P.max_fix_per_k) {
+    if (total_fix >= RC_P.max_fix_per_k) {
         const int nw = (len + 63) >> 6;
         for (int c = 0; c <= nw; ++c) {
             const uint64_t f = w.ballot64(c << 6, len, [&](int q) { return S.base[q] != 4 && S.best[q] != -1; });
@@ -1258,7 +1346,7 @@
         w.sync();
         int bad = 0;
         for (int i = w.lane; i < kcnt; i += W::STRIDE)
-            if (rc_popc64(rc_window(S.m_a, i, k)) + rc_popc64(rc_window(S.m_t, i, k)) > 2 * P.max_fix_per_k) bad = 1;
+            if (rc_popc64(rc_window(S.m_a, i, k)) + rc_popc64(rc_window(S.m_t, i, k)) > 2 * RC_P.max_fix_per_k) bad = 1;
         if (w.reduce_add(bad)) return -1;
     }
 
diff --git a/rcorrector_amd/csrc/rc_correct_kernel.h b/rcorrector_amd/csrc/rc_correct_kernel.h
--- a/rcorrector_amd/csrc/rc_correct_kernel.h
+++ b/rcorrector_amd/csrc/rc_correct_kernel.h
@@ -5,412 +5,6 @@
 
 #include "rc_internal.h"
 #include "rc_device.h"
-
-template <bool PROF, bool TRACE = false, bool SORT_REGS = true, int KT_ = 0>
-struct DevWaveT {
-    static const int STRIDE = 64;
-    static constexpr int KT = KT_;
-    int lane;
-    unsigned long long t_last = 0;
-    int cur_phase = 0;
-    unsigned long long *acc = nullptr;
-#ifdef RC_EXP_ROUNDS
-    int rounds = 0;
-    __device__ __forceinline__ void stat(int i, int v)
-    {
-        if (i == 3) rounds += v;
-    }
-#else
-    int rounds = 0, rounds_max = 0;
-    long long rounds_sum = 0;
-    long long stv[10] = {0, 0, 0, 0, 0, 0, 0, 0, 0, 0};
-    __device__ __forceinline__ void stat(int i, int v)
-    {
-        if (PROF && i == 3) rounds += v;
-        if (PROF && i != 3 && i < 10) stv[i] += v;
-    }
-#endif
-    int32_t *tr = nullptr;
-    int tr_cap = 0;
-    __device__ __forceinline__ void trace_passed()
-    {
-        if (TRACE && lane == 0) tr[0] |= 1;
-    }
-    __device__ __forceinline__ void trace_iter(int strong, int trust)
-    {
-        if (TRACE) {
-            const int it = uni(tr[1]);
-            if (lane == 0) {
-                if (it < tr_cap) {
-                    int32_t *e = tr + 2 + (size_t)it * RC_TRACE_WORDS;
-                    e[0] = strong;
-                    e[1] = trust;
-                    e[2] = 0;
-                    e[3] = 0;
-                }
-                tr[1] = it + 1;
-            }
-            sync();
-        }
-    }
-    __device__ __forceinline__ void trace_strong(const unsigned char *strongb, int len)
-    {
-        if (TRACE) {
-            const int it = uni(tr[1]) - 1;
-            if (it >= 0 && it < tr_cap) {
-                int32_t *e = tr + 2 + (size_t)it * RC_TRACE_WORDS;
-                for (int c = 0; c < RC_MAX_READ_LENGTH / 64; ++c) {
-                    const uint64_t m = ballot64(c << 6, len, [&](int q) { return strongb[q] != 0; });
-                    if (lane == 0) {
-                        e[4 + 2 * c] = (int32_t)(uint32_t)m;
-                        e[5 + 2 * c] = (int32_t)(uint32_t)(m >> 32);
-                    }
-                }
-                if (lane == 0) e[2] = 1;
-            }
-            sync();
-        }
-    }
-    __device__ __forceinline__ int uni(int x) { return __builtin_amdgcn_readfirstlane(x); }
-    __device__ __forceinline__ uint64_t uni64(uint64_t x)
-    {
-        const uint32_t lo = (uint32_t)__builtin_amdgcn_readfirstlane((int)(uint32_t)x);
-        const uint32_t hi = (uint32_t)__builtin_amdgcn_readfirstlane((int)(uint32_t)(x >> 32));
-        return ((uint64_t)hi << 32) | lo;
-    }
-    __device__ __forceinline__ void phase(int id)
-    {
-        if (id < 8) asm volatile("" : "+v"(lane));
-        if (PROF) {
-            unsigned long long t = __builtin_readcyclecounter();
-            if (lane == 0) acc[cur_phase] += t - t_last;
-            t_last = t;
-            cur_phase = id;
-        }
-    }
-    rc_table_view T;
-    int k;
-    rc_frame *stack;
-
-    __device__ __forceinline__ void sync()
-    {
-        __builtin_amdgcn_fence(__ATOMIC_RELEASE, "wavefront");
-        __builtin_amdgcn_wave_barrier();
-        __builtin_amdgcn_fence(__ATOMIC_ACQUIRE, "wavefront");
-    }
-
-    template <class F>
-    __device__ __forceinline__ uint64_t ballot64(int base, int n, F pred)
-    {
-        const int i = base + lane;
-        bool p = false;
-        if (i < n) p = pred(i);
-        return __ballot(p);
-    }
-    template <class F>
-    __device__ __forceinline__ void for_lanes64(int base, int n, F body)
-    {
-        const int i = base + lane;
-        if (i < n) body(i, lane);
-    }
-
-    __device__ __forceinline__ int reduce_add(int x)
-    {
-#pragma unroll
-        for (int o = 32; o > 0; o >>= 1) x += __shfl_xor(x, o, 64);
-        return __builtin_amdgcn_readfirstlane(x);
-    }
-
-    template <bool MAX>
-    __device__ __forceinline__ uint32_t wave_minmax_u32(uint32_t x)
-    {
-        auto op = [](uint32_t a, uint32_t b) { return MAX ? (a > b ? a : b) : (a < b ? a : b); };
-        x = op(x, (uint32_t)__builtin_amdgcn_update_dpp(0, (int)x, 0xB1, 0xF, 0xF, true));
-        x = op(x, (uint32_t)__builtin_amdgcn_update_dpp(0, (int)x, 0x4E, 0xF, 0xF, true));
-        x = op(x, (uint32_t)__builtin_amdgcn_update_dpp(0, (int)x, 0x141, 0xF, 0xF, true));
-        x = op(x, (uint32_t)__builtin_amdgcn_update_dpp(0, (int)x, 0x140, 0xF, 0xF, true));
-        const uint32_t r0 = (uint32_t)__builtin_amdgcn_readlane((int)x, 0), r1 = (uint32_t)__builtin_amdgcn_readlane((int)x, 16);
-        const uint32_t r2 = (uint32_t)__builtin_amdgcn_readlane((int)x, 32), r3 = (uint32_t)__builtin_amdgcn_readlane((int)x, 48);
-        return op(op(r0, r1), op(r2, r3));
-    }
-    __device__ __forceinline__ uint32_t wave_min_u32(uint32_t x) { return wave_minmax_u32<false>(x); }
-    __device__ __forceinline__ uint32_t wave_max_u32(uint32_t x) { return wave_minmax_u32<true>(x); }
-
-    __device__ __forceinline__ void prefix_min(const int *in, int *out, int j0, int n)
-    {
-        const bool live = lane >= j0 && lane < n;
-        int x = live ? in[lane] : 2147483647;
-        auto step = [&](int y) { x = y < x ? y : x; };
-        step(__builtin_amdgcn_update_dpp(2147483647, x, 0x111, 0xF, 0xF, false));
-        step(__builtin_amdgcn_update_dpp(2147483647, x, 0x112, 0xF, 0xF, false));
-        step(__builtin_amdgcn_update_dpp(2147483647, x, 0x114, 0xF, 0xF, false));
-        step(__builtin_amdgcn_update_dpp(2147483647, x, 0x118, 0xF, 0xF, false));
-        if (n > 16) {
-            const int r0 = __builtin_amdgcn_readlane(x, 15), r1 = __builtin_amdgcn_readlane(x, 31), r2 = __builtin_amdgcn_readlane(x, 47);
-            const int m01 = r0 < r1 ? r0 : r1, m012 = m01 < r2 ? m01 : r2;
-            const int row = lane >> 4;
-            const int before = row == 0 ? 2147483647 : (row == 1 ? r0 : (row == 2 ? m01 : m012));
-            x = before < x ? before : x;
-        }
-        if (live) out[lane] = x;
-    }
-    __device__ __forceinline__ int min_range(const int *a, int lo, int hi)
-    {
-        const int i = lo + lane;
-        const uint32_t x = i < hi ? ((uint32_t)a[i] ^ 0x80000000u) : 0xFFFFFFFFu;
-        return (int)(wave_min_u32(x) ^ 0x80000000u);
-    }
-
-    uint32_t n_req = 0;
-    uint32_t n_probe = 0, n_absent = 0;
-    __device__ __forceinline__ int get(rc_kmer km, int dir = 0)
-    {
-        if (km.inv != -1) return 0;
-        const uint64_t rv = rc_revcomp(km.code, KT ? KT : k);
-        const uint64_t canon = rv < km.code ? rv : km.code;
-        const int c = rc_table_lookup_o<true, true>(T, canon, dir > 0 ? km.code : (dir < 0 ? rv : canon), PROF ? &n_req : nullptr);
-        if (PROF) {
-            ++n_probe;
-            n_absent += c == 0 ? 1u : 0u;
-        }
-        return c;
-    }
-
-    __device__ __forceinline__ int lookup(uint64_t code) { return rc_table_lookup(T, rc_canonical(code, KT ? KT : k), PROF ? &n_req : nullptr); }
-
-    template <int E>
-    __device__ __forceinline__ void bitonic_regs(int *a, int n)
-    {
-        int x[E];
-#pragma unroll
-        for (int e = 0; e < E; ++e) {
-            const int g = e * 64 + lane;
-            x[e] = g < n ? a[g] : 2147483647;
-        }
-#pragma unroll
-        for (int size = 2; size <= E * 64; size <<= 1) {
-#pragma unroll
-            for (int stride = size >> 1; stride > 0; stride >>= 1) {
-                if (stride >= 64) {
-#pragma unroll
-                    for (int e = 0; e < E; ++e) {
-                        const int pe = e ^ (stride >> 6);
-                        if (pe > e) {
-                            const bool up = ((e * 64) & size) == 0;
-                            const int lo = x[e] < x[pe] ? x[e] : x[pe];
-                            const int hi = x[e] < x[pe] ? x[pe] : x[e];
-                            x[e] = up ? lo : hi;
-                            x[pe] = up ? hi : lo;
-                        }
-                    }
-                } else {
-#pragma unroll
-                    for (int e = 0; e < E; ++e) {
-                        const int g = e * 64 + lane;
-                        const int y = __shfl_xor(x[e], stride, 64);
-                        const bool up = (g & size) == 0;
-                        const bool lower = (lane & stride) == 0;
-                        const int lo = x[e] < y ? x[e] : y;
-                        const int hi = x[e] < y ? y : x[e];
-                        x[e] = (up == lower) ? lo : hi;
-                    }
-                }
-            }
-        }
-        sync();
-#pragma unroll
-        for (int e = 0; e < E; ++e) {
-            const int g = e * 64 + lane;
-            if (g < n) a[g] = x[e];
-        }
-        sync();
-    }
-
-    __device__ __forceinline__ void sort(int *a, int n)
-    {
-        if (SORT_REGS) {
-            if (n <= 64) return bitonic_regs<1>(a, n);
-            if (n <= 128) return bitonic_regs<2>(a, n);
-            if (n <= 256) return bitonic_regs<4>(a, n);
-        }
-        int n2 = 1;
-        while (n2 < n) n2 <<= 1;
-        for (int i = n + lane; i < n2; i += 64) a[i] = 2147483647;
-        sync();
-        for (int size = 2; size <= n2; size <<= 1) {
-            for (int stride = size >> 1; stride > 0; stride >>= 1) {
-                for (int t = lane; t < (n2 >> 1); t += 64) {
-                    const int pos = 2 * t - (t & (stride - 1));
-                    const int par = pos + stride;
-                    const bool up = (pos & size) == 0;
-                    const int x = a[pos], y = a[par];
-                    if ((x > y) == up) {
-                        a[pos] = y;
-                        a[par] = x;
-                    }
-                }
-                sync();
-            }
-        }
-    }
-
-    uint32_t *lstack = nullptr;
-    int lstack_n = 0;
-    static constexpr int FRAME_DWORDS = (int)(sizeof(rc_frame) / 4);
-    __device__ __forceinline__ void stack_push(int sp, const rc_frame &f)
-    {
-        if (sp < lstack_n) {
-            if (lane == 0) {
-                uint32_t *d = lstack + sp * FRAME_DWORDS;
-                d[0] = (uint32_t)f.code;
-                d[1] = (uint32_t)(f.code >> 32);
-                d[2] = (uint32_t)f.inv;
-                d[3] = (uint32_t)f.pos;
-                d[4] = (uint32_t)f.t;
-                d[5] = (uint32_t)f.threshold;
-                d[6] = (uint32_t)f.fix_cnt;
-                d[7] = (uint32_t)f.bottleneck;
-                d[8] = (uint32_t)f.cnt.c0;
-                d[9] = (uint32_t)f.cnt.c1;
-                d[10] = (uint32_t)f.cnt.c2;
-                d[11] = (uint32_t)f.cnt.c3;
-                d[12] = (uint32_t)f.mask;
-            }
-            sync();
-            return;
-        }
-        if (lane == 0) stack[sp] = f;
-        __threadfence_block();
-    }
-    __device__ __forceinline__ void stack_top(int idx, rc_frame &f)
-    {
-        static_assert(sizeof(rc_frame) == 56 && offsetof(rc_frame, mask) == 48, "rc_frame layout");
-        uint32_t d[13];
-        if (idx < lstack_n) {
-            const uint32_t *p = lstack + idx * FRAME_DWORDS;
-#pragma unroll
-            for (int q = 0; q < 13; ++q) d[q] = p[q];
-        } else {
-            const uint32_t *p = reinterpret_cast<const uint32_t *>(stack + idx);
-#pragma unroll
-            for (int q = 0; q < 13; ++q) d[q] = __hip_atomic_load(p + q, __ATOMIC_RELAXED, __HIP_MEMORY_SCOPE_WORKGROUP);
-        }
-        f.code = ((uint64_t)(uint32_t)uni((int)d[1]) << 32) | (uint32_t)uni((int)d[0]);
-        f.inv = uni((int)d[2]);
-        f.pos = uni((int)d[3]);
-        f.t = uni((int)d[4]);
-        f.threshold = uni((int)d[5]);
-        f.fix_cnt = uni((int)d[6]);
-        f.bottleneck = uni((int)d[7]);
-        f.cnt.c0 = uni((int)d[8]);
-        f.cnt.c1 = uni((int)d[9]);
-        f.cnt.c2 = uni((int)d[10]);
-        f.cnt.c3 = uni((int)d[11]);
-        f.mask = uni((int)d[12]);
-    }
-    __device__ __forceinline__ void stack_set_mask(int idx, int mask)
-    {
-        if (idx < lstack_n) {
-            if (lane == 0) lstack[idx * FRAME_DWORDS + 12] = (uint32_t)mask;
-            sync();
-            return;
-        }
-        if (lane == 0) stack[idx].mask = mask;
-        __threadfence_block();
-    }
-};
-typedef DevWaveT<false> DevWave;
-
-#ifndef RC_DEQUEUE
-#define RC_DEQUEUE 8
-#endif
-#define RC_META_WORDS 6
-
-struct rc_lds_layout {
-    int cap, cap2;
-    size_t o_counts, o_v, o_isl, o_seg, o_base, o_path, o_best, o_strongb, o_polya, o_qual, o_masks, o_spec, o_pk, o_meta, total;
-    int mask_words;
-};
-
-static __host__ __device__ constexpr inline int rc_seg_capacity(int cap) { return cap <= 192 ? 20 : cap / 6 + 4; }
-
-static __host__ __device__ constexpr inline rc_lds_layout rc_layout(int cap)
-{
-    rc_lds_layout L{};
-    L.cap = cap;
-    int c2 = 64;
-    while (c2 < cap) c2 <<= 1;
-    L.cap2 = c2;
-    const int nseg = rc_seg_capacity(cap);
-    const int nisl = cap / 3 + 2;
-    size_t o = 0;
-    L.mask_words = cap / 64 + 2;
-    L.o_masks = o;
-    o += (size_t)L.mask_words * 8 * 5;
-    L.o_spec = o;
-    o += (size_t)RC_SPEC_ENTRIES * 4 + (size_t)RC_SPEC * (8 + 4 + 4 * 4) + 16 + (size_t)(4 + RC_MEMO_MAX) * 4;
-    L.o_pk = o;
-    o += (size_t)(cap / 16 + 4) * 4;
-    L.o_meta = o;
-    o += (size_t)RC_DEQUEUE * RC_META_WORDS * 4;
-    L.o_counts = o;
-    o += (size_t)cap * 4;
-    L.o_v = o;
-    o += (size_t)c2 * 4;
-    L.o_seg = o;
-    o += (size_t)nseg * sizeof(rc_segment);
-    if ((size_t)nisl * sizeof(rc_island) <= (size_t)RC_SPEC_ENTRIES * 4 + (size_t)RC_SPEC * 8) {
-        L.o_isl = L.o_spec;
-    } else {
-        L.o_isl = o;
-        o += (size_t)nisl * sizeof(rc_island);
-    }
-    o = (o + 15) & ~(size_t)15;
-    L.o_base = o;
-    o += cap;
-    L.o_path = o;
-    o += cap;
-    L.o_best = o;
-    o += cap;
-    L.o_strongb = o;
-    o += cap;
-    L.o_polya = o;
-    o += cap;
-    L.o_qual = o;
-    o += cap;
-    L.total = (o + 15) & ~(size_t)15;
-    return L;
-}
-
-__device__ __forceinline__ void rc_carve(uint8_t *lds, const rc_lds_layout &L, rc_read_state &S)
-{
-    S.counts = reinterpret_cast<int *>(lds + L.o_counts);
-    S.v = reinterpret_cast<int *>(lds + L.o_v);
-    S.seg = reinterpret_cast<rc_segment *>(lds + L.o_seg);
-    S.isl = reinterpret_cast<rc_island *>(lds + L.o_isl);
-    S.base = lds + L.o_base;
-    S.path = reinterpret_cast<signed char *>(lds + L.o_path);
-    S.best = reinterpret_cast<signed char *>(lds + L.o_best);
-    S.strongb = lds + L.o_strongb;
-    S.polya = lds + L.o_polya;
-    S.qual = reinterpret_cast<signed char *>(lds + L.o_qual);
-    uint64_t *mm = reinterpret_cast<uint64_t *>(lds + L.o_masks);
-    S.m_a = mm;
-    S.m_t = mm + L.mask_words;
-    S.m_n = mm + 2 * L.mask_words;
-    S.m_inv = mm + 3 * L.mask_words;
-    S.m_x = mm + 4 * L.mask_words;
-    S.pk = reinterpret_cast<uint32_t *>(lds + L.o_pk);
-    S.spec_code = reinterpret_cast<uint64_t *>(lds + L.o_spec);
-    S.spec_cnt = reinterpret_cast<int *>(lds + L.o_spec + RC_SPEC * 8);
-    S.spec_inv = S.spec_cnt + RC_SPEC_ENTRIES;
-    S.spec_ret = S.spec_inv + RC_SPEC;
-    S.spec_keep = S.spec_ret + RC_SPEC;
-    S.spec_thr = S.spec_keep + RC_SPEC;
-    S.spec_mask = S.spec_thr + RC_SPEC;
-    S.spec_meta = S.spec_mask + RC_SPEC;
-    S.memo = S.spec_meta + 4;
-}
 
 struct rc_kernel_args {
     rc_table_view T;
@@ -445,6 +39,388 @@
     int tier_lo, tier_hi;
     int pair_override;
 };
+
+template <bool PROF, bool TRACE = false, bool SORT_REGS = true, int KT_ = 0, bool KARG = false, int TL_ = 0>
+struct DevWaveT {
+    static const int STRIDE = 64;
+    static constexpr int KT = KT_;
+    int lane;
+    typedef const __attribute__((address_space(4))) rc_kernel_args *karg_ptr;
+    __device__ __forceinline__ karg_ptr args() const
+    {
+        karg_ptr p = (karg_ptr)__builtin_amdgcn_kernarg_segment_ptr();
+        asm volatile("" : "+s"(p));
+        return p;
+    }
+    __device__ __forceinline__ const rc_run_params &params(const rc_run_params &P) const
+    {
+        if (!KARG) return P;
+        return *(const rc_run_params *)&args()->P;
+    }
+    __device__ __forceinline__ rc_table_view table() const
+    {
+        if (!KARG) return T;
+        karg_ptr a = args();
+        rc_table_view t;
+        t.buckets = a->T.buckets;
+        t.nb_home = a->T.nb_home;
+        t.nbuckets_alloc = a->T.nbuckets_alloc;
+        t.layout = TL_ != 0 ? 1 : a->T.layout;
+        t.k = KT != 0 ? KT : a->T.k;
+        t.ext = TL_ == 1 ? 0 : a->T.ext;
+        t.filter = a->T.filter;
+        t.filter_words = a->T.filter_words;
+        t.filter_kind = a->T.filter_kind;
+        t.filter_all = a->T.filter_all;
+        return t;
+    }
+    __device__ __forceinline__ int run_k() const { return KT ? KT : (KARG ? args()->P.k : k); }
+    __device__ __forceinline__ rc_frame *hbm_stack() const
+    {
+        if (!KARG) return stack;
+        karg_ptr a = args();
+        return a->stack + (size_t)blockIdx.x * a->stack_frames;
+    }
+    unsigned long long t_last = 0;
+    int cur_phase = 0;
+    unsigned long long *acc = nullptr;
+#ifdef RC_EXP_ROUNDS
+    int rounds = 0;
+    __device__ __forceinline__ void stat(int i, int v)
+    {
+        if (i == 3) rounds += v;
+    }
+#else
+    int rounds = 0, rounds_max = 0;
+    long long rounds_sum = 0;
+    long long stv[10] = {0, 0, 0, 0, 0, 0, 0, 0, 0, 0};
+    __device__ __forceinline__ void stat(int i, int v)
+    {
+        if (PROF && i == 3) rounds += v;
+        if (PROF && i != 3 && i < 10) stv[i] += v;
+    }
+#endif
+    int32_t *tr = nullptr;
+    int tr_cap = 0;
+    __device__ __forceinline__ void trace_passed()
+    {
+        if (TRACE && lane == 0) tr[0] |= 1;
+    }
+    __device__ __forceinline__ void trace_iter(int strong, int trust)
+    {
+        if (TRACE) {
+            const int it = uni(tr[1]);
+            if (lane == 0) {
+                if (it < tr_cap) {
+                    int32_t *e = tr + 2 + (size_t)it * RC_TRACE_WORDS;
+                    e[0] = strong;
+                    e[1] = trust;
+                    e[2] = 0;
+                    e[3] = 0;
+                }
+                tr[1] = it + 1;
+            }
+            sync();
+        }
+    }
+    __device__ __forceinline__ void trace_strong(const unsigned char *strongb, int len)
+    {
+        if (TRACE) {
+            const int it = uni(tr[1]) - 1;
+            if (it >= 0 && it < tr_cap) {
+                int32_t *e = tr + 2 + (size_t)it * RC_TRACE_WORDS;
+                for (int c = 0; c < RC_MAX_READ_LENGTH / 64; ++c) {
+                    const uint64_t m = ballot64(c << 6, len, [&](int q) { return strongb[q] != 0; });
+                    if (lane == 0) {
+                        e[4 + 2 * c] = (int32_t)(uint32_t)m;
+                        e[5 + 2 * c] = (int32_t)(uint32_t)(m >> 32);
+                    }
+                }
+                if (lane == 0) e[2] = 1;
+            }
+            sync();
+        }
+    }
+    __device__ __forceinline__ int uni(int x) { return __builtin_amdgcn_readfirstlane(x); }
+    __device__ __forceinline__ uint64_t uni64(uint64_t x)
+    {
+        const uint32_t lo = (uint32_t)__builtin_amdgcn_readfirstlane((int)(uint32_t)x);
+        const uint32_t hi = (uint32_t)__builtin_amdgcn_readfirstlane((int)(uint32_t)(x >> 32));
+        return ((uint64_t)hi << 32) | lo;
+    }
+    __device__ __forceinline__ void phase(int id)
+    {
+        if (id < 8) asm volatile("" : "+v"(lane));
+        if (PROF) {
+            unsigned long long t = __builtin_readcyclecounter();
+            if (lane == 0) acc[cur_phase] += t - t_last;
+            t_last = t;
+            cur_phase = id;
+        }
+    }
+    rc_table_view T;
+    int k;
+    rc_frame *stack;
+
+    __device__ __forceinline__ void sync()
+    {
+        __builtin_amdgcn_fence(__ATOMIC_RELEASE, "wavefront");
+        __builtin_amdgcn_wave_barrier();
+        __builtin_amdgcn_fence(__ATOMIC_ACQUIRE, "wavefront");
+    }
+
+    template <class F>
+    __device__ __forceinline__ uint64_t ballot64(int base, int n, F pred)
+    {
+        const int i = base + lane;
+        bool p = false;
+        if (i < n) p = pred(i);
+        return __ballot(p);
+    }
+    template <class F>
+    __device__ __forceinline__ void for_lanes64(int base, int n, F body)
+    {
+        const int i = base + lane;
+        if (i < n) body(i, lane);
+    }
+
+    __device__ __forceinline__ int reduce_add(int x)
+    {
+#pragma unroll
+        for (int o = 32; o > 0; o >>= 1) x += __shfl_xor(x, o, 64);
+        return __builtin_amdgcn_readfirstlane(x);
+    }
+
+    template <bool MAX>
+    __device__ __forceinline__ uint32_t wave_minmax_u32(uint32_t x)
+    {
+        auto op = [](uint32_t a, uint32_t b) { return MAX ? (a > b ? a : b) : (a < b ? a : b); };
+        x = op(x, (uint32_t)__builtin_amdgcn_update_dpp(0, (int)x, 0xB1, 0xF, 0xF, true));
+        x = op(x, (uint32_t)__builtin_amdgcn_update_dpp(0, (int)x, 0x4E, 0xF, 0xF, true));
+        x = op(x, (uint32_t)__builtin_amdgcn_update_dpp(0, (int)x, 0x141, 0xF, 0xF, true));
+        x = op(x, (uint32_t)__builtin_amdgcn_update_dpp(0, (int)x, 0x140, 0xF, 0xF, true));
+        const uint32_t r0 = (uint32_t)__builtin_amdgcn_readlane((int)x, 0), r1 = (uint32_t)__builtin_amdgcn_readlane((int)x, 16);
+        const uint32_t r2 = (uint32_t)__builtin_amdgcn_readlane((int)x, 32), r3 = (uint32_t)__builtin_amdgcn_readlane((int)x, 48);
+        return op(op(r0, r1), op(r2, r3));
+    }
+    __device__ __forceinline__ uint32_t wave_min_u32(uint32_t x) { return wave_minmax_u32<false>(x); }
+    __device__ __forceinline__ uint32_t wave_max_u32(uint32_t x) { return wave_minmax_u32<true>(x); }
+
+    __device__ __forceinline__ void prefix_min(const int *in, int *out, int j0, int n)
+    {
+        const bool live = lane >= j0 && lane < n;
+        int x = live ? in[lane] : 2147483647;
+        auto step = [&](int y) { x = y < x ? y : x; };
+        step(__builtin_amdgcn_update_dpp(2147483647, x, 0x111, 0xF, 0xF, false));
+        step(__builtin_amdgcn_update_dpp(2147483647, x, 0x112, 0xF, 0xF, false));
+        step(__builtin_amdgcn_update_dpp(2147483647, x, 0x114, 0xF, 0xF, false));
+        step(__builtin_amdgcn_update_dpp(2147483647, x, 0x118, 0xF, 0xF, false));
+        if (n > 16) {
+            const int r0 = __builtin_amdgcn_readlane(x, 15), r1 = __builtin_amdgcn_readlane(x, 31), r2 = __builtin_amdgcn_readlane(x, 47);
+            const int m01 = r0 < r1 ? r0 : r1, m012 = m01 < r2 ? m01 : r2;
+            const int row = lane >> 4;
+            const int before = row == 0 ? 2147483647 : (row == 1 ? r0 : (row == 2 ? m01 : m012));
+            x = before < x ? before : x;
+        }
+        if (live) out[lane] = x;
+    }
+    __device__ __forceinline__ int min_range(const int *a, int lo, int hi)
+    {
+        const int i = lo + lane;
+        const uint32_t x = i < hi ? ((uint32_t)a[i] ^ 0x80000000u) : 0xFFFFFFFFu;
+        return (int)(wave_min_u32(x) ^ 0x80000000u);
+    }
+
+    uint32_t n_req = 0;
+    uint32_t n_probe = 0, n_absent = 0;
+    __device__ __forceinline__ int get(rc_kmer km, int dir = 0)
+    {
+        if (km.inv != -1) return 0;
+        const uint64_t rv = rc_revcomp(km.code, run_k());
+        const uint64_t canon = rv < km.code ? rv : km.code;
+        const int c = rc_table_lookup_o<true, true>(table(), canon, dir > 0 ? km.code : (dir < 0 ? rv : canon), PROF ? &n_req : nullptr);
+        if (PROF) {
+            ++n_probe;
+            n_absent += c == 0 ? 1u : 0u;
+        }
+        return c;
+    }
+
+    __device__ __forceinline__ int lookup(uint64_t code) { return rc_table_lookup(table(), rc_canonical(code, run_k()), PROF ? &n_req : nullptr); }
+
+    template <int E>
+    __device__ __forceinline__ void bitonic_regs(int *a, int n)
+    {
+        int x[E];
+#pragma unroll
+        for (int e = 0; e < E; ++e) {
+            const int g = e * 64 + lane;
+            x[e] = g < n ? a[g] : 2147483647;
+        }
+#pragma unroll
+        for (int size = 2; size <= E * 64; size <<= 1) {
+#pragma unroll
+            for (int stride = size >> 1; stride > 0; stride >>= 1) {
+                if (stride >= 64) {
+#pragma unroll
+                    for (int e = 0; e < E; ++e) {
+                        const int pe = e ^ (stride >> 6);
+                        if (pe > e) {
+                            const bool up = ((e * 64) & size) == 0;
+                            const int lo = x[e] < x[pe] ? x[e] : x[pe];
+                            const int hi = x[e] < x[pe] ? x[pe] : x[e];
+                            x[e] = up ? lo : hi;
+                            x[pe] = up ? hi : lo;
+                        }
+                    }
+                } else {
+#pragma unroll
+                    for (int e = 0; e < E; ++e) {
+                        const int g = e * 64 + lane;
+                        const int y = __shfl_xor(x[e], stride, 64);
+                        const bool up = (g & size) == 0;
+                        const bool lower = (lane & stride) == 0;
+                        const int lo = x[e] < y ? x[e] : y;
+                        const int hi = x[e] < y ? y : x[e];
+                        x[e] = (up == lower) ? lo : hi;
+                    }
+                }
+            }
+        }
+        sync();
+#pragma unroll
+        for (int e = 0; e < E; ++e) {
+            const int g = e * 64 + lane;
+            if (g < n) a[g] = x[e];
+        }
+        sync();
+    }
+
+    __device__ __forceinline__ void sort(int *a, int n)
+    {
+        if (SORT_REGS) {
+            if (n <= 64) return bitonic_regs<1>(a, n);
+            if (n <= 128) return bitonic_regs<2>(a, n);
+            if (n <= 256) return bitonic_regs<4>(a, n);
+        }
+        int n2 = 1;
+        while (n2 < n) n2 <<= 1;
+        for (int i = n + lane; i < n2; i += 64) a[i] = 2147483647;
+        sync();
+        for (int size = 2; size <= n2; size <<= 1) {
+            for (int stride = size >> 1; stride > 0; stride >>= 1) {
+                for (int t = lane; t < (n2 >> 1); t += 64) {
+                    const int pos = 2 * t - (t & (stride - 1));
+                    const int par = pos + stride;
+                    const bool up = (pos & size) == 0;
+                    const int x = a[pos], y = a[par];
+                    if ((x > y) == up) {
+                        a[pos] = y;
+                        a[par] = x;
+                    }
+                }
+                sync();
+            }
+        }
+    }
+
+    uint32_t *lstack = nullptr;
+    int lstack_n = 0;
+    static constexpr int FRAME_DWORDS = (int)(sizeof(rc_frame) / 4);
+    __device__ __forceinline__ void stack_push(int sp, const rc_frame &f)
+    {
+        if (sp < lstack_n) {
+            if (lane == 0) {
+                uint32_t *d = lstack + sp * FRAME_DWORDS;
+                d[0] = (uint32_t)f.code;
+                d[1] = (uint32_t)(f.code >> 32);
+                d[2] = (uint32_t)f.inv;
+                d[3] = (uint32_t)f.pos;
+                d[4] = (uint32_t)f.t;
+                d[5] = (uint32_t)f.threshold;
+                d[6] = (uint32_t)f.fix_cnt;
+                d[7] = (uint32_t)f.bottleneck;
+                d[8] = (uint32_t)f.cnt.c0;
+                d[9] = (uint32_t)f.cnt.c1;
+                d[10] = (uint32_t)f.cnt.c2;
+                d[11] = (uint32_t)f.cnt.c3;
+                d[12] = (uint32_t)f.mask;
+            }
+            sync();
+            return;
+        }
+        if (lane == 0) hbm_stack()[sp] = f;
+        __threadfence_block();
+    }
+    __device__ __forceinline__ void stack_top(int idx, rc_frame &f)
+    {
+        static_assert(sizeof(rc_frame) == 56 && offsetof(rc_frame, mask) == 48, "rc_frame layout");
+        uint32_t d[13];
+        if (idx < lstack_n) {
+            const uint32_t *p = lstack + idx * FRAME_DWORDS;
+#pragma unroll
+            for (int q = 0; q < 13; ++q) d[q] = p[q];
+        } else {
+            const uint32_t *p = reinterpret_cast<const uint32_t *>(hbm_stack() + idx);
+#pragma unroll
+            for (int q = 0; q < 13; ++q) d[q] = __hip_atomic_load(p + q, __ATOMIC_RELAXED, __HIP_MEMORY_SCOPE_WORKGROUP);
+        }
+        f.code = ((uint64_t)(uint32_t)uni((int)d[1]) << 32) | (uint32_t)uni((int)d[0]);
+        f.inv = uni((int)d[2]);
+        f.pos = uni((int)d[3]);
+        f.t = uni((int)d[4]);
+        f.threshold = uni((int)d[5]);
+        f.fix_cnt = uni((int)d[6]);
+        f.bottleneck = uni((int)d[7]);
+        f.cnt.c0 = uni((int)d[8]);
+        f.cnt.c1 = uni((int)d[9]);
+        f.cnt.c2 = uni((int)d[10]);
+        f.cnt.c3 = uni((int)d[11]);
+        f.mask = uni((int)d[12]);
+    }
+    __device__ __forceinline__ void stack_set_mask(int idx, int mask)
+    {
+        if (idx < lstack_n) {
+            if (lane == 0) lstack[idx * FRAME_DWORDS + 12] = (uint32_t)mask;
+            sync();
+            return;
+        }
+        if (lane == 0) hbm_stack()[idx].mask = mask;
+        __threadfence_block();
+    }
+};
+typedef DevWaveT<false> DevWave;
+
+__device__ __forceinline__ void rc_carve(uint8_t *lds, const rc_lds_layout &L, rc_read_state &S)
+{
+    S.counts = reinterpret_cast<int *>(lds + L.o_counts);
+    S.v = reinterpret_cast<int *>(lds + L.o_v);
+    S.seg = reinterpret_cast<rc_segment *>(lds + L.o_seg);
+    S.isl = reinterpret_cast<rc_island *>(lds + L.o_isl);
+    S.base = lds + L.o_base;
+    S.path = reinterpret_cast<signed char *>(lds + L.o_path);
+    S.best = reinterpret_cast<signed char *>(lds + L.o_best);
+    S.strongb = lds + L.o_strongb;
+    S.polya = lds + L.o_polya;
+    S.qual = reinterpret_cast<signed char *>(lds + L.o_qual);
+    uint64_t *mm = reinterpret_cast<uint64_t *>(lds + L.o_masks);
+    S.m_a = mm;
+    S.m_t = mm + L.mask_words;
+    S.m_n = mm + 2 * L.mask_words;
+    S.m_inv = mm + 3 * L.mask_words;
+    S.m_x = mm + 4 * L.mask_words;
+    S.pk = reinterpret_cast<uint32_t *>(lds + L.o_pk);
+    S.spec_code = reinterpret_cast<uint64_t *>(lds + L.o_spec);
+    S.spec_cnt = reinterpret_cast<int *>(lds + L.o_spec + RC_SPEC * 8);
+    S.spec_inv = S.spec_cnt + RC_SPEC_ENTRIES;
+    S.spec_ret = S.spec_inv + RC_SPEC;
+    S.spec_keep = S.spec_ret + RC_SPEC;
+    S.spec_thr = S.spec_keep + RC_SPEC;
+    S.spec_mask = S.spec_thr + RC_SPEC;
+    S.spec_meta = S.spec_mask + RC_SPEC;
+    S.memo = S.spec_meta + 4;
+}
+
 __device__ __forceinline__ int rc_unit_max_len(const rc_kernel_args &A, uint32_t r, int len)
 {
     if (A.mode == 0) return len;
@@ -483,49 +459,50 @@
 }
 
 template <int CAP, bool PROF, bool TRACE, int KT = 0, int TL = 0>
-__global__ __launch_bounds__(64, rc_k3_waves(CAP)) void k_correct(rc_kernel_args A)
+__global__ __launch_bounds__(64, rc_k3_waves(CAP)) void k_correct(rc_kernel_args)
 {
     constexpr rc_lds_layout L = rc_layout(CAP);
+    static_assert(CAP > 192 || L.total <= 5120, "k_correct<192>: 32 one-wave blocks per CU (8 waves per SIMD) need <= 5 120 B of LDS each");
     __shared__ __attribute__((aligned(16))) uint8_t lds[L.total + (PROF ? 128 : 0)];
     rc_read_state S;
     rc_carve(lds, L, S);
-    typedef DevWaveT<PROF, TRACE, false, KT> W;
+    typedef DevWaveT<PROF, TRACE, false, KT, true, TL> W;
     W w;
     w.lane = threadIdx.x;
-    w.tr_cap = A.trace_cap;
+#define RC_KA (*(const rc_kernel_args *)w.args())
+    w.tr_cap = TRACE ? RC_KA.trace_cap : 0;
     if (PROF) {
         w.acc = reinterpret_cast<unsigned long long *>(lds + L.total);
         if (w.lane < 16) w.acc[w.lane] = 0;
         w.sync();
         w.t_last = __builtin_readcyclecounter();
     }
-    w.T = A.T;
-    if (TL != 0) w.T.layout = 1;
-    if (TL == 1) w.T.ext = 0;
-    if (KT != 0) w.T.k = KT;
-    w.k = A.P.k;
-    w.stack = A.stack + (size_t)blockIdx.x * A.stack_frames;
     w.lstack = reinterpret_cast<uint32_t *>(S.v);
     w.lstack_n = (int)((size_t)L.cap2 * 4 / sizeof(rc_frame));
-    if (PROF && w.lane == 0) atomicMin(A.phase_cycles + 8, (unsigned long long)wall_clock64());
-    const int n_sections = A.n_work ? RC_WORK_CLASSES : 1;
-    int section = 0;
-    uint32_t n_work = A.n_work ? (uint32_t)__builtin_amdgcn_readfirstlane((int)A.n_work[0]) : A.n;
-    const uint32_t *list = A.worklist;
-    uint32_t *heads = A.work;
-    uint32_t chunk_lo = 0, chunk_hi = 0, chunk_base = 0;
+    if (PROF && w.lane == 0) atomicMin(RC_KA.phase_cycles + 8, (unsigned long long)wall_clock64());
+    int32_t *D = reinterpret_cast<int32_t *>(lds + L.o_desc);
     uint32_t *meta = reinterpret_cast<uint32_t *>(lds + L.o_meta);
-    int head = (int)(blockIdx.x % RC_HEADS), heads_done = 0;
+    D[RC_D_CHUNK_LO] = 0;
+    D[RC_D_CHUNK_HI] = 0;
+    D[RC_D_CHUNK_BASE] = 0;
+    D[RC_D_QUEUE] = rc_desc_queue(0, (int)(blockIdx.x % RC_HEADS), 0);
+    w.sync();
     for (;;) {
-        if (chunk_lo >= chunk_hi) {
+        uint32_t chunk_lo = (uint32_t)w.uni(D[RC_D_CHUNK_LO]);
+        if (chunk_lo >= (uint32_t)w.uni(D[RC_D_CHUNK_HI])) {
+            const int n_sections = RC_KA.n_work ? RC_WORK_CLASSES : 1;
+            const int q = w.uni(D[RC_D_QUEUE]);
+            int section = rc_desc_section(q), head = rc_desc_head(q), heads_done = rc_desc_heads_done(q);
+            uint32_t chunk_hi = 0;
             bool got = false;
             for (;;) {
+                const uint32_t n_work = RC_KA.n_work ? (uint32_t)__builtin_amdgcn_readfirstlane((int)RC_KA.n_work[section]) : RC_KA.n;
                 while (heads_done < RC_HEADS) {
                     const uint32_t lo = (uint32_t)(((uint64_t)n_work * (uint32_t)head) / RC_HEADS);
                     const uint32_t hi = (uint32_t)(((uint64_t)n_work * (uint32_t)(head + 1)) / RC_HEADS);
                     uint32_t r0 = hi - lo;
                     if (hi > lo) {
-                        if (w.lane == 0) r0 = atomicAdd(heads + head * 32, (uint32_t)RC_DEQUEUE);
+                        if (w.lane == 0) r0 = atomicAdd(RC_KA.work + section * (RC_HEADS * 32) + head * 32, (uint32_t)RC_DEQUEUE);
                         r0 = (uint32_t)__builtin_amdgcn_readfirstlane((int)r0);
                     }
                     if (r0 < hi - lo) {
@@ -538,20 +515,20 @@
                     ++heads_done;
                 }
                 if (got || ++section >= n_sections) break;
-                n_work = (uint32_t)__builtin_amdgcn_readfirstlane((int)A.n_work[section]);
-                list = A.worklist + (size_t)section * A.work_stride;
-                heads = A.work + section * (RC_HEADS * 32);
                 head = (int)(blockIdx.x % RC_HEADS);
                 heads_done = 0;
             }
             if (!got) {
-                if (PROF && w.lane == 0) atomicMin(A.phase_cycles + 9, (unsigned long long)wall_clock64());
+                if (PROF && w.lane == 0) atomicMin(RC_KA.phase_cycles + 9, (unsigned long long)wall_clock64());
                 break;
             }
-            chunk_base = chunk_lo;
+            D[RC_D_CHUNK_HI] = (int32_t)chunk_hi;
+            D[RC_D_CHUNK_BASE] = (int32_t)chunk_lo;
+            D[RC_D_QUEUE] = rc_desc_queue(section, head, heads_done);
             if ((uint32_t)w.lane < chunk_hi - chunk_lo) {
+                const rc_kernel_args &A = RC_KA;
                 uint32_t ri = chunk_lo + (uint32_t)w.lane;
-                if (list) ri = list[ri];
+                if (A.worklist) ri = (A.worklist + (size_t)section * A.work_stride)[ri];
                 uint32_t *mw = meta + w.lane * RC_META_WORDS;
                 mw[0] = ri;
                 mw[1] = A.off[ri];
@@ -568,57 +545,61 @@
             }
             w.sync();
         }
-        const int ci = (int)(chunk_lo - chunk_base);
-        ++chunk_lo;
-        const uint32_t *me = meta + ci * RC_META_WORDS;
-        const uint32_t r = (uint32_t)w.uni((int)me[0]);
-        const uint32_t o = (uint32_t)w.uni((int)me[1]);
+        const uint32_t *me = meta + (int)(chunk_lo - (uint32_t)w.uni(D[RC_D_CHUNK_BASE])) * RC_META_WORDS;
+        D[RC_D_CHUNK_LO] = (int32_t)(chunk_lo + 1);
+        D[RC_D_META] = (int32_t)(me - meta);
         w.phase(0);
         if (TRACE) {
-            w.tr = A.trace + (size_t)r * (2 + (size_t)A.trace_cap * RC_TRACE_WORDS);
+            w.tr = RC_KA.trace + (size_t)(uint32_t)w.uni((int)me[0]) * (2 + (size_t)RC_KA.trace_cap * RC_TRACE_WORDS);
             if (w.lane == 0) w.tr[0] = w.tr[1] = 0;
             w.sync();
         }
 #if defined(RC_EXP_STOP) && RC_EXP_STOP == 0
-        if (w.lane == 0) A.ret[r] = (int)o;
+        if (w.lane == 0) RC_KA.ret[w.uni((int)me[0])] = w.uni((int)me[1]);
         continue;
 #endif
-        rc_load_read(w, A, S, o, w.uni((int)(me[2] - o) - 1), w.lane, true);
+        {
+            const uint32_t o = (uint32_t)w.uni((int)me[1]);
+            rc_load_read(w, RC_KA, S, o, w.uni((int)(me[2] - o) - 1), w.lane, true);
+        }
 #if defined(RC_EXP_STOP) && RC_EXP_STOP == 1
-        if (w.lane == 0) A.ret[r] = (int)S.m_inv[0] + (int)S.pk[1] + S.counts[5] + S.qual[7];
+        if (w.lane == 0) RC_KA.ret[w.uni((int)me[0])] = (int)S.m_inv[0] + (int)S.pk[1] + S.counts[5] + S.qual[7];
         w.sync();
         continue;
 #endif
         int strong0, info0;
-        if (A.fused_front_end) {
+        if (RC_KA.fused_front_end) {
             w.phase(1);
-            strong0 = rc_front_end(w, S, A.P, &info0);
+            strong0 = rc_front_end(w, S, w.params(RC_KA.P), &info0);
         } else {
             strong0 = w.uni((int)me[3]);
             info0 = w.uni((int)me[4]);
         }
-        int pair_t = A.pair_override;
-        if (A.mode != 0) pair_t = rc_min(strong0, w.uni((int)me[5]));
+        int pair_t = RC_KA.pair_override;
+        if (RC_KA.mode != 0) pair_t = rc_min(strong0, w.uni((int)me[5]));
         w.phase(1);
-        if (!A.fused_front_end && S.kcnt > 0 && !(info0 & 4)) rc_polya_flags(w, S, RC_K(A.P));
+        if (!RC_KA.fused_front_end && S.kcnt > 0 && !(info0 & 4)) rc_polya_flags(w, S, RC_K(RC_KA.P));
 #if defined(RC_EXP_STOP) && RC_EXP_STOP == 2
-        if (w.lane == 0) A.ret[r] = (int)S.polya[3] + pair_t;
+        if (w.lane == 0) RC_KA.ret[w.uni((int)me[0])] = (int)S.polya[3] + pair_t;
         w.sync();
         continue;
 #endif
-        const int ret = rc_correct_read(w, S, A.P, pair_t, strong0, info0);
+        const int ret = rc_correct_read(w, S, w.params(RC_KA.P), pair_t, strong0, info0);
+        const uint32_t *me2 = meta + w.uni(D[RC_D_META]);
+        const uint32_t r = (uint32_t)w.uni((int)me2[0]), o = (uint32_t)w.uni((int)me2[1]);
 #if defined(RC_EXP_STOP) && (RC_EXP_STOP == 3 || RC_EXP_STOP == 4 || RC_EXP_STOP == 5)
-        if (w.lane == 0) A.ret[r] = ret + S.best[3] + S.seg[0].from;
+        if (w.lane == 0) RC_KA.ret[r] = ret + S.best[3] + S.seg[0].from;
         w.sync();
         continue;
 #endif
         w.phase(6);
         w.sync();
         if (ret > 0) {
+            uint8_t *seq = RC_KA.seq;
             for (int i = w.lane; i < S.len; i += 64) {
                 const int f = S.best[i];
                 if (f != -1) {
-                    A.seq[o + i] = (uint8_t)("ACGT"[f]);
+                    seq[o + i] = (uint8_t)("ACGT"[f]);
                     S.base[i] = (unsigned char)f;
                 }
             }
@@ -626,8 +607,9 @@
             rc_pack_read(w, S);
         }
         int l, m, h;
-        rc_kmer_info(w, S, A.P, ret, &l, &m, &h);
+        rc_kmer_info(w, S, w.params(RC_KA.P), ret, &l, &m, &h);
         if (w.lane == 0) {
+            const rc_kernel_args &A = RC_KA;
             A.ret[r] = ret;
 #ifdef RC_EXP_ROUNDS
             A.l[r] = w.rounds;
@@ -642,7 +624,7 @@
         w.phase(7);
 #ifndef RC_EXP_ROUNDS
         if (PROF) {
-            if (A.rounds_out && w.lane == 0) A.rounds_out[r] = w.rounds;
+            if (RC_KA.rounds_out && w.lane == 0) RC_KA.rounds_out[r] = w.rounds;
             w.rounds_sum += w.rounds;
             w.rounds_max = w.rounds > w.rounds_max ? w.rounds : w.rounds_max;
             w.rounds = 0;
@@ -650,25 +632,28 @@
 #endif
     }
     if (PROF && w.lane == 0) {
+        unsigned long long *pc = RC_KA.phase_cycles;
         w.phase(7);
-        for (int i = 0; i < 8; ++i) atomicAdd(A.phase_cycles + i, w.acc[i]);
-        for (int i = 8; i < 16; ++i) atomicAdd(A.phase_cycles + 8 + i, w.acc[i]);
-        atomicMax(A.phase_cycles + 10, (unsigned long long)wall_clock64());
+        for (int i = 0; i < 8; ++i) atomicAdd(pc + i, w.acc[i]);
+        for (int i = 8; i < 16; ++i) atomicAdd(pc + 8 + i, w.acc[i]);
+        atomicMax(pc + 10, (unsigned long long)wall_clock64());
 #ifndef RC_EXP_ROUNDS
-        atomicAdd(A.phase_cycles + 11, (unsigned long long)w.rounds_sum);
-        atomicMax(A.phase_cycles + 12, (unsigned long long)w.rounds_max);
+        atomicAdd(pc + 11, (unsigned long long)w.rounds_sum);
+        atomicMax(pc + 12, (unsigned long long)w.rounds_max);
         for (int i = 0; i < 10; ++i)
-            if (i != 3) atomicAdd(A.phase_cycles + 24 + i, (unsigned long long)w.stv[i]);
+            if (i != 3) atomicAdd(pc + 24 + i, (unsigned long long)w.stv[i]);
 #endif
     }
     if (PROF) {
         const int req = w.reduce_add((int)w.n_req), prb = w.reduce_add((int)w.n_probe), abs_ = w.reduce_add((int)w.n_absent);
         if (w.lane == 0) {
-            atomicAdd(A.phase_cycles + 13, (unsigned long long)(uint32_t)req);
-            atomicAdd(A.phase_cycles + 14, (unsigned long long)(uint32_t)prb);
-            atomicAdd(A.phase_cycles + 15, (unsigned long long)(uint32_t)abs_);
-        }
-    }
+            unsigned long long *pc = RC_KA.phase_cycles;
+            atomicAdd(pc + 13, (unsigned long long)(uint32_t)req);
+            atomicAdd(pc + 14, (unsigned long long)(uint32_t)prb);
+            atomicAdd(pc + 15, (unsigned long long)(uint32_t)abs_);
+        }
+    }
+#undef RC_KA
 }
 
 typedef void (*rc_k3_launcher)(dim3 grid, hipStream_t stream, const rc_kernel_args &A);
```

Result: slower. 363.0 million (-1.2%).
